# ju-liu/krylov

Hardware: AMD Instinct MI355X
Metric: CG iters/sec + SpMV GB/s (fp64, n=10M, nnz=150M); GMRES(30) iters/sec (higher is better)
Workload: dtype f64; 1 GPU; krylov.cg, 3-D 15-point stencil 216^3, one RHS per GPU, tol=0 fixed iterations; n=10077696, nnz=149770936, index=int32, rhs_per_gpu=1, parallelism=rhs-shard x1, launch=one GPU

## Files before the change

include/krylov_hip.h:

```cpp
#ifndef KRYLOV_HIP_H
#define KRYLOV_HIP_H

#include <stdint.h>

#ifdef __cplusplus
extern "C" {
#endif

typedef struct kry_ctx kry_ctx;
typedef struct kry_csr kry_csr;
typedef struct kry_vec kry_vec;
typedef struct kry_cg kry_cg;
typedef struct kry_gmres kry_gmres;
typedef struct kry_minres kry_minres;
typedef struct kry_comm kry_comm;
typedef struct kry_prog kry_prog;
typedef struct kry_tri kry_tri;
typedef struct kry_precond kry_precond;

enum { KRY_F32 = 1, KRY_F64 = 2 };
enum { KRY_I32 = 1, KRY_I64 = 2 };

enum {
  KRY_OK = 0,
  KRY_EINVAL = -1,
  KRY_ENOMEM = -2,
  KRY_EDEVICE = -3,
  KRY_EINVARIANT = -4,
  KRY_EUNSUPPORTED = -5,
  KRY_ESINGULAR = -6,
  KRY_ENONFINITE = -7,
  KRY_ECOMM = -8
};

int kry_version(void);
const char *kry_last_error(void);
const char *kry_build_id(void);
int kry_device_count(int *count);
int kry_ctx_create(int device, kry_ctx **out);
int kry_ctx_destroy(kry_ctx *ctx);
int kry_ctx_synchronize(kry_ctx *ctx);

int kry_mem_stats(int64_t *out);
int kry_mem_release(void);

int kry_csr_create(kry_ctx *ctx, int64_t n, int64_t nnz, const void *indptr,
                   const void *indices, const void *data, int dtype, int itype,
                   kry_csr **out);
int kry_csr_destroy(kry_csr *A);
int kry_csr_create_like(kry_ctx *ctx, const kry_csr *like, int64_t n, int64_t nnz, const void *indptr,
                        const void *indices, const void *data, int dtype, int itype, kry_csr **out);
int kry_csr_create_ex(kry_ctx *ctx, int64_t n, int64_t nnz, const void *indptr, const void *indices,
                      const void *data, int dtype, int itype, int renumber, kry_csr **out);
int kry_csr_permute(kry_ctx *ctx, const kry_csr *A, const kry_vec *src, kry_vec *dst, int to_operator);
int kry_csr_compare(const kry_csr *A, const kry_csr *B, int64_t *out);
int kry_spmv_op(kry_ctx *ctx, kry_csr *A, kry_vec *x, kry_vec *y);
int kry_rcm_plan(int64_t n, int64_t nnz, const void *indptr, const void *indices, int itype, int64_t wlimit,
                 int64_t *info, int32_t *perm);
int kry_rcm_device(kry_ctx *ctx, int64_t n, int64_t nnz, const int32_t *indptr, const int32_t *indices, int64_t wlimit,
                   int64_t *info, int32_t *perm);
int kry_rs_plan(int64_t n, int64_t nnz, const void *indptr, const void *indices, int itype, int64_t *info,
                int32_t *widths, uint32_t *colrank);
int kry_csr_layout(int64_t n, const void *indptr, int itype, int64_t *nslices,
                   int64_t *nslots, int64_t *nirregular);
int kry_dia_plan(int64_t n, int64_t nnz, const void *indptr, const void *indices, int itype, int64_t *info,
                 int32_t *widths, int32_t *offsets, uint64_t *masks);
int kry_dia_uniform_plan(int64_t n, int64_t nnz, const void *indptr, const void *indices, const void *data, int dtype,
                         int itype, int64_t *info, int32_t *flags, void *values);
int kry_pair_plan(int64_t n, int64_t nnz, const void *indptr, const void *indices, int itype, int64_t *info,
                  int32_t *widths, int32_t *cbase, uint16_t *deltas);
int kry_cb_plan(int64_t n, int64_t nnz, const void *indptr, const void *indices, int itype, int64_t *info,
                int64_t *gptr);
#define KRY_CSR_INFO_LEN 16
int kry_csr_info_n(const kry_csr *A, int64_t *info, int32_t len);
int kry_csr_info(const kry_csr *A, int64_t *info);

int kry_vec_create(kry_ctx *ctx, int64_t n, int32_t k, int dtype, kry_vec **out);
int kry_vec_destroy(kry_vec *v);
int kry_vec_upload(kry_vec *v, const void *host);
int kry_vec_download(kry_vec *v, void *host);

int kry_spmv(kry_ctx *ctx, kry_csr *A, kry_vec *x, kry_vec *y);
int kry_dot(kry_ctx *ctx, kry_vec *x, kry_vec *y, kry_vec *w, double *out);
int kry_axpy(kry_ctx *ctx, const double *alpha, kry_vec *x, kry_vec *y);
int kry_vec_lincomb(kry_ctx *ctx, int form, kry_vec *z, kry_vec *x, kry_vec *y, kry_vec *w,
                    const double *a, const double *b);
int kry_prog_create(kry_ctx *ctx, int32_t nregs, int32_t k, int32_t cap, kry_prog **out);
int kry_prog_destroy(kry_prog *p);
int kry_prog_set(kry_prog *p, int32_t r, const double *vals);
int kry_prog_get(kry_prog *p, int32_t r, double *vals);
int kry_prog_begin(kry_prog *p);
int kry_prog_end(kry_prog *p, int32_t steps, int32_t *done, int32_t *midstep, double *rows);
int kry_prog_scalar(kry_prog *p, int32_t op, int32_t d, int32_t a, int32_t b, int32_t c, int32_t e, double value,
                    int32_t step);
int kry_prog_dot(kry_prog *p, kry_vec *x, kry_vec *y, kry_vec *w, int32_t d, int32_t step);
int kry_prog_lincomb(kry_prog *p, int32_t form, kry_vec *z, kry_vec *x, kry_vec *y, kry_vec *w, int32_t ra, double sa,
                     int32_t rb, double sb, int32_t step);
int kry_prog_spmv(kry_prog *p, kry_csr *A, kry_vec *x, kry_vec *y, int32_t step);
int kry_prog_check(kry_prog *p, int32_t r, int32_t mode, int32_t step);
int kry_prog_rowscale(kry_prog *p, int32_t mul, kry_vec *z, kry_vec *x, kry_vec *d, int32_t step);
int kry_prog_permute(kry_prog *p, const kry_csr *A, const kry_vec *src, kry_vec *dst, int32_t to_operator,
                     int32_t step);
int kry_prog_trisolve(kry_prog *p, const kry_tri *T, const kry_vec *y, kry_vec *x, int32_t step);

int kry_tri_plan(int64_t n, int64_t nnz, const void *indptr, const void *indices, int itype, int lower, int64_t *info,
                 int32_t *level, int32_t *order, int32_t *launch, int32_t *widths);
int kry_tri_create(kry_ctx *ctx, int64_t n, int64_t nnz, const void *indptr, const void *indices, const void *data,
                   int dtype, int itype, int lower, kry_tri **out);
int kry_tri_plan_ordered(int64_t n, int64_t nnz, const void *indptr, const void *indices, int itype, int lower,
                         const int32_t *rank, int64_t *info, int32_t *level, int32_t *order, int32_t *launch,
                         int32_t *widths);
int kry_tri_create_ordered(kry_ctx *ctx, int64_t n, int64_t nnz, const void *indptr, const void *indices,
                           const void *data, int dtype, int itype, int lower, const int32_t *rank, kry_tri **out);
int kry_color_plan(int64_t n, int64_t nnz, const void *indptr, const void *indices, int itype, int64_t *info,
                   int32_t *color, int32_t *perm);
int kry_tri_destroy(kry_tri *T);
int kry_tri_info(const kry_tri *T, int64_t *info);
int kry_tri_solve(kry_ctx *ctx, const kry_tri *T, const kry_vec *y, kry_vec *x);

int kry_ilu0_plan(int64_t n, int64_t nnz, const void *indptr, const void *indices, int itype, int64_t *info,
                  int32_t *level, int32_t *order, int32_t *launch, int64_t *diag);
int kry_isai_lower(kry_ctx *ctx, int64_t n, int64_t nnz, const void *indptr, const void *indices, const void *data,
                   int dtype, int itype, void *values, int64_t *info);
int kry_precond_add_isai(kry_precond *P, const kry_csr *W, const kry_csr *T, int32_t sweeps, const kry_vec *scale);
int kry_ilu0_factor(kry_ctx *ctx, int64_t n, int64_t nnz, const void *indptr, const void *indices, const void *data,
                    int dtype, int itype, void *values, int64_t *info);
int kry_precond_create(kry_ctx *ctx, int64_t n, int dtype, kry_precond **out);
int kry_precond_destroy(kry_precond *P);
int kry_precond_add_tri(kry_precond *P, const kry_tri *T);
int kry_precond_add_scale(kry_precond *P, const kry_vec *d);
int kry_precond_fuse(kry_precond *P);
int kry_precond_info(const kry_precond *P, int64_t *info);
int kry_precond_apply(kry_ctx *ctx, const kry_precond *P, const kry_vec *x, kry_vec *y);
int kry_prog_precond(kry_prog *p, const kry_precond *P, const kry_vec *x, kry_vec *y, int32_t step);
int kry_cg_set_precond(kry_cg *s, int32_t slot, const kry_precond *P);
int kry_gmres_set_precond(kry_gmres *s, int32_t slot, const kry_precond *P);
int kry_minres_set_precond(kry_minres *s, int32_t slot, const kry_precond *P);

int kry_lartg(kry_ctx *ctx, int64_t count, int dtype, const void *f, const void *g,
              void *c, void *s, void *r);

int kry_cg_create(kry_ctx *ctx, kry_csr *A, int32_t k, int dtype, kry_cg **out);
int kry_cg_destroy(kry_cg *s);
int kry_cg_set_preconditioners(kry_cg *s, kry_csr *M, kry_csr *Ml);
int kry_cg_start(kry_cg *s, kry_vec *b, kry_vec *x0, kry_vec *w, double *rho0);
int kry_cg_set_criterion(kry_cg *s, const double *criterion);
int kry_cg_run(kry_cg *s, int32_t max_steps, int32_t *steps_done, double *resnorms);
int kry_cg_preferred_chunk(kry_cg *s, int32_t *steps);
int kry_cg_path(kry_cg *s, int32_t *info);
int kry_cg_update_path(kry_cg *s, int32_t *info);
int kry_cg_defer_info(kry_cg *s, int32_t *D, int64_t *bytes);
int kry_cg_residual(kry_cg *s, double *resnorm);
int kry_cg_get(kry_cg *s, int which, void *host);
int kry_cg_scalars(kry_cg *s, double *out);

int kry_gmres_create(kry_ctx *ctx, kry_csr *A, int32_t k, int dtype, int32_t maxiter,
// ... 50 lines not shown
```

krylov_amd/_lib.py:

```python
import atexit
import ctypes
import os
import threading
import weakref

import numpy as np

from .errors import exception_for

_HERE = os.path.dirname(os.path.abspath(__file__))
LIB_PATH = os.path.join(_HERE, "libkrylov_hip.so")
if os.environ.get("KRYLOV_LIB"):
    LIB_PATH = os.environ["KRYLOV_LIB"]

KRY_F32, KRY_F64 = 1, 2
KRY_I32, KRY_I64 = 1, 2

KRY_OK = 0
KRY_EINVAL = -1
KRY_ENOMEM = -2
KRY_EDEVICE = -3
KRY_EINVARIANT = -4
KRY_EUNSUPPORTED = -5
KRY_ESINGULAR = -6
KRY_ENONFINITE = -7
KRY_ECOMM = -8

PROF_SPMV, PROF_UPDATE, PROF_MGS, PROF_OTHER = 0, 1, 2, 3

if not os.path.exists(LIB_PATH):
    raise ImportError(
        f"{LIB_PATH} is missing: build it with `python -c 'import __graft_entry__ as g; g.build()'` "
        "or `make -C krylov_amd/csrc` (hipcc, gfx950). krylov_amd has no CPU fallback."
    )

lib = ctypes.CDLL(LIB_PATH)
HOST_ONLY = not hasattr(lib, "kry_ctx_create")

_vp = ctypes.c_void_p
_pvp = ctypes.POINTER(ctypes.c_void_p)
_i32 = ctypes.c_int32
_i64 = ctypes.c_int64
_int = ctypes.c_int
_dp = ctypes.POINTER(ctypes.c_double)
_ip32 = ctypes.POINTER(ctypes.c_int32)
_ip64 = ctypes.POINTER(ctypes.c_int64)

_SIGNATURES = {
    "kry_device_count": [ctypes.POINTER(_int)],
    "kry_ctx_create": [_int, _pvp],
    "kry_ctx_destroy": [_vp],
    "kry_ctx_synchronize": [_vp],
    "kry_csr_create": [_vp, _i64, _i64, _vp, _vp, _vp, _int, _int, _pvp],
    "kry_csr_destroy": [_vp],
    "kry_csr_create_ex": [_vp, _i64, _i64, _vp, _vp, _vp, _int, _int, _int, _pvp],
    "kry_csr_create_like": [_vp, _vp, _i64, _i64, _vp, _vp, _vp, _int, _int, _pvp],
    "kry_csr_permute": [_vp, _vp, _vp, _vp, _int],
    "kry_csr_compare": [_vp, _vp, _ip64],
    "kry_spmv_op": [_vp, _vp, _vp, _vp],
    "kry_rcm_plan": [ctypes.c_int64, ctypes.c_int64, _vp, _vp, _int, ctypes.c_int64, _ip64, _vp],
    "kry_rs_plan": [ctypes.c_int64, ctypes.c_int64, _vp, _vp, _int, _ip64, _vp, _vp],
    "kry_rcm_device": [_vp, ctypes.c_int64, ctypes.c_int64, _vp, _vp, ctypes.c_int64, _ip64, _vp],
    "kry_csr_layout": [_i64, _vp, _int, _ip64, _ip64, _ip64],
    "kry_dia_plan": [ctypes.c_int64, ctypes.c_int64, _vp, _vp, _int, _ip64, _vp, _vp, _vp],
    "kry_dia_uniform_plan": [ctypes.c_int64, ctypes.c_int64, _vp, _vp, _vp, _int, _int, _ip64, _vp, _vp],
    "kry_pair_plan": [ctypes.c_int64, ctypes.c_int64, _vp, _vp, _int, _ip64, _vp, _vp, _vp],
    "kry_cb_plan": [ctypes.c_int64, ctypes.c_int64, _vp, _vp, _int, _ip64, _vp],
    "kry_csr_info": [_vp, _ip64],
    "kry_csr_info_n": [_vp, _ip64, _i32],
    "kry_vec_create": [_vp, _i64, _i32, _int, _pvp],
    "kry_vec_destroy": [_vp],
    "kry_vec_upload": [_vp, _vp],
    "kry_vec_download": [_vp, _vp],
    "kry_spmv": [_vp, _vp, _vp, _vp],
    "kry_dot": [_vp, _vp, _vp, _vp, _dp],
    "kry_axpy": [_vp, _dp, _vp, _vp],
    "kry_lartg": [_vp, _i64, _int, _vp, _vp, _vp, _vp, _vp],
    "kry_cg_create": [_vp, _vp, _i32, _int, _pvp],
    "kry_cg_destroy": [_vp],
    "kry_cg_start": [_vp, _vp, _vp, _vp, _dp],
    "kry_cg_set_criterion": [_vp, _dp],
    "kry_cg_run": [_vp, _i32, _ip32, _dp],
    "kry_cg_preferred_chunk": [_vp, _ip32],
    "kry_cg_path": [_vp, _ip32],
    "kry_cg_update_path": [_vp, _ip32],
    "kry_cg_defer_info": [_vp, _ip32, _ip64],
    "kry_minres_update_path": [_vp, _ip32],
    "kry_cg_residual": [_vp, _dp],
    "kry_cg_get": [_vp, _int, _vp],
    "kry_cg_scalars": [_vp, _dp],
    "kry_vec_lincomb": [_vp, _int, _vp, _vp, _vp, _vp, _dp, _dp],
    "kry_cg_set_preconditioners": [_vp, _vp, _vp],
    "kry_gmres_set_preconditioners": [_vp, _vp, _vp, _vp],
    "kry_minres_set_preconditioners": [_vp, _vp, _vp, _vp],
    "kry_gmres_create": [_vp, _vp, _i32, _int, _i32, _i32, _pvp],
    "kry_gmres_destroy": [_vp],
    "kry_gmres_start": [_vp, _vp, _vp, _vp, _dp],
    "kry_gmres_set_criterion": [_vp, _dp],
    "kry_gmres_run": [_vp, _i32, _ip32, _dp, _ip32],
    "kry_trsv_upper": [_vp, _i32, _i32, ctypes.c_int, _dp, _dp, _dp],
    "kry_householder": [_vp, _vp, _vp, _dp],
    "kry_gmres_solution": [_vp],
    "kry_gmres_residual": [_vp, _dp],
    "kry_gmres_get": [_vp, _int, _vp],
    "kry_gmres_xk_device": [_vp, _vp],
    "kry_gmres_path": [_vp, _ip32],
    "kry_minres_create": [_vp, _vp, _i32, _int, _pvp],
    "kry_minres_destroy": [_vp],
    "kry_minres_start": [_vp, _vp, _vp, _vp, _dp],
    "kry_minres_set_criterion": [_vp, _dp],
    "kry_minres_run": [_vp, _i32, _ip32, _dp, _ip32],
    "kry_minres_residual": [_vp, _dp],
    "kry_minres_get": [_vp, _int, _vp],
    "kry_comm_unique_id": [_vp],
    "kry_comm_create": [_vp, _i32, _i32, _vp, _pvp],
    "kry_comm_destroy": [_vp],
    "kry_comm_abort": [_vp],
    "kry_comm_create_all": [_vp, _i32, _vp],
    "kry_comm_allreduce": [_vp, _dp, _i32],
    "kry_comm_info": [_vp, _vp, _vp],
    "kry_cg_attach_comm": [_vp, _vp, _i32, _i32],
    "kry_gmres_attach_comm": [_vp, _vp, _i32, _i32],
    "kry_minres_attach_comm": [_vp, _vp, _i32, _i32],
    "kry_timer_start": [_vp],
    "kry_timer_stop": [_vp, _dp],
    "kry_profile_enable": [_vp, _int],
    "kry_profile_select": [_vp, ctypes.c_uint32, ctypes.c_int32],
    "kry_profile_read": [_vp, _int, _ip64, _dp],
    "kry_prog_create": [_vp, _i32, _i32, _i32, _pvp],
    "kry_prog_destroy": [_vp],
    "kry_prog_set": [_vp, _i32, _dp],
    "kry_prog_get": [_vp, _i32, _dp],
    "kry_prog_begin": [_vp],
    "kry_prog_end": [_vp, _i32, _ip32, _ip32, _dp],
    "kry_prog_scalar": [_vp, _i32, _i32, _i32, _i32, _i32, _i32, ctypes.c_double, _i32],
    "kry_prog_dot": [_vp, _vp, _vp, _vp, _i32, _i32],
    "kry_prog_lincomb": [_vp, _i32, _vp, _vp, _vp, _vp, _i32, ctypes.c_double, _i32, ctypes.c_double, _i32],
    "kry_prog_spmv": [_vp, _vp, _vp, _vp, _i32],
    "kry_prog_check": [_vp, _i32, _i32, _i32],
    "kry_prog_rowscale": [_vp, _i32, _vp, _vp, _vp, _i32],
    "kry_prog_permute": [_vp, _vp, _vp, _vp, _i32, _i32],
    "kry_prog_trisolve": [_vp, _vp, _vp, _vp, _i32],
    "kry_tri_plan": [ctypes.c_int64, ctypes.c_int64, _vp, _vp, _int, _int, _ip64, _vp, _vp, _vp, _vp],
    "kry_tri_create": [_vp, _i64, _i64, _vp, _vp, _vp, _int, _int, _int, _pvp],
    "kry_tri_plan_ordered": [ctypes.c_int64, ctypes.c_int64, _vp, _vp, _int, _int, _vp, _ip64, _vp, _vp, _vp, _vp],
    "kry_tri_create_ordered": [_vp, _i64, _i64, _vp, _vp, _vp, _int, _int, _int, _vp, _pvp],
    "kry_color_plan": [ctypes.c_int64, ctypes.c_int64, _vp, _vp, _int, _ip64, _vp, _vp],
    "kry_tri_destroy": [_vp],
# ... 52 lines not shown

def dtype_code(dt):
    dt = np.dtype(dt)
    if dt == np.float64:
        return KRY_F64
    if dt == np.float32:
        return KRY_F32
    raise TypeError(f"the MI355X path computes in float32/float64, not {dt}")


def itype_code(dt):
    dt = np.dtype(dt)
    if dt == np.int32:
        return KRY_I32
    if dt == np.int64:
        return KRY_I64
    raise TypeError(f"CSR index arrays must be int32 or int64, not {dt}")


def ptr(a):
    assert a.flags.c_contiguous
    return ctypes.c_void_p(a.ctypes.data)


def dptr(a):
    assert a.dtype == np.float64 and a.flags.c_contiguous
    return a.ctypes.data_as(_dp)


def device_count():
    c = _int(0)
    check(lib.kry_device_count(ctypes.byref(c)))
    return c.value


def memory_stats():
    out = np.zeros(6, dtype=np.int64)
    check(lib.kry_mem_stats(out.ctypes.data_as(_ip64)))
    keys = ("bytes_in_use", "bytes_cached", "reuses", "device_mallocs", "retire_syncs", "enabled")
    return {k: int(v) for k, v in zip(keys, out)}


def empty_cache():
    check(lib.kry_mem_release())


def dia_plan(indptr, indices):
    indptr = np.ascontiguousarray(indptr)
    indices = np.ascontiguousarray(indices, dtype=indptr.dtype)
    n, nnz = indptr.shape[0] - 1, indices.shape[0]
    info = np.zeros(4, dtype=np.int64)
    ip64 = info.ctypes.data_as(ctypes.POINTER(ctypes.c_int64))
    check(lib.kry_dia_plan(n, nnz, ptr(indptr), ptr(indices), itype_code(indptr.dtype), ip64, None, None, None))
    if not info[0]:
        return None
    cols = int(info[2]) // 128
    widths = np.zeros(int(info[1]), dtype=np.int32)
    offsets = np.zeros(cols, dtype=np.int32)
    masks = np.zeros(2 * cols, dtype=np.uint64)
    check(lib.kry_dia_plan(n, nnz, ptr(indptr), ptr(indices), itype_code(indptr.dtype), ip64, ptr(widths),
                           ptr(offsets), ptr(masks)))
    return {"slices": int(info[1]), "slots": int(info[2]), "max_width": int(info[3]), "widths": widths,
            "offsets": offsets, "masks": masks}


def dia_uniform_plan(indptr, indices, data):
    indptr = np.ascontiguousarray(indptr)
    indices = np.ascontiguousarray(indices, dtype=indptr.dtype)
    data = np.ascontiguousarray(data)
    n, nnz = indptr.shape[0] - 1, indices.shape[0]
    assert data.shape[0] == nnz
    info = np.zeros(3, dtype=np.int64)
    ip64 = info.ctypes.data_as(ctypes.POINTER(ctypes.c_int64))
    args = (n, nnz, ptr(indptr), ptr(indices), ptr(data), dtype_code(data.dtype), itype_code(indptr.dtype), ip64)
    check(lib.kry_dia_uniform_plan(*args, None, None))
    if not info[0]:
        return None
    flags = np.zeros(int(info[1]), dtype=np.int32)
    values = np.zeros(int(info[1]), dtype=data.dtype)
    check(lib.kry_dia_uniform_plan(*args, ptr(flags), ptr(values)))
    return {"cols": int(info[1]), "uniform": int(info[2]), "flags": flags, "values": values}


def pair_plan(indptr, indices):
    indptr = np.ascontiguousarray(indptr)
    indices = np.ascontiguousarray(indices, dtype=indptr.dtype)
    n, nnz = indptr.shape[0] - 1, indices.shape[0]
    info = np.zeros(4, dtype=np.int64)
    ip64 = info.ctypes.data_as(ctypes.POINTER(ctypes.c_int64))
    check(lib.kry_pair_plan(n, nnz, ptr(indptr), ptr(indices), itype_code(indptr.dtype), ip64, None, None, None))
    if not info[0]:
        return None
    slots = int(info[2])
    widths = np.zeros(int(info[1]), dtype=np.int32)
    cbase = np.zeros(slots // 128, dtype=np.int32)
    deltas = np.zeros(slots, dtype=np.uint16)
    check(lib.kry_pair_plan(n, nnz, ptr(indptr), ptr(indices), itype_code(indptr.dtype), ip64, ptr(widths),
                            ptr(cbase), ptr(deltas)))
    return {"slices": int(info[1]), "slots": slots, "max_width": int(info[3]), "widths": widths, "cbase": cbase,
            "deltas": deltas}


def cb_plan(indptr, indices):
    indptr = np.ascontiguousarray(indptr)
    indices = np.ascontiguousarray(indices, dtype=indptr.dtype)
    n, nnz = indptr.shape[0] - 1, indices.shape[0]
    info = np.zeros(4, dtype=np.int64)
    ip64 = info.ctypes.data_as(ctypes.POINTER(ctypes.c_int64))
    check(lib.kry_cb_plan(n, nnz, ptr(indptr), ptr(indices), itype_code(indptr.dtype), ip64, None))
    if not info[0]:
        return None
    nb, ng = int(info[1]), int(info[3])
    gptr = np.zeros(nb * ng + 1, dtype=np.int64)
    check(lib.kry_cb_plan(n, nnz, ptr(indptr), ptr(indices), itype_code(indptr.dtype), ip64, ptr(gptr)))
    return {"nb": nb, "cols": int(info[2]), "ng": ng, "gptr": gptr}


def rcm_plan(indptr, indices, wlimit=0):
    indptr = np.ascontiguousarray(indptr)
    indices = np.ascontiguousarray(indices, dtype=indptr.dtype)
    n, nnz = indptr.shape[0] - 1, indices.shape[0]
    info = np.zeros(2, dtype=np.int64)
    perm = np.zeros(max(n, 1), dtype=np.int32)
    check(lib.kry_rcm_plan(n, nnz, ptr(indptr), ptr(indices), itype_code(indptr.dtype), int(wlimit),
                           info.ctypes.data_as(ctypes.POINTER(ctypes.c_int64)), ptr(perm)))
    if not info[0]:
        return None
    return perm[:n], int(info[1])


def rs_plan(indptr, indices):
    indptr = np.ascontiguousarray(indptr)
    indices = np.ascontiguousarray(indices, dtype=indptr.dtype)
    n, nnz = indptr.shape[0] - 1, indices.shape[0]
    info = np.zeros(4, dtype=np.int64)
    ip64 = info.ctypes.data_as(ctypes.POINTER(ctypes.c_int64))
    check(lib.kry_rs_plan(n, nnz, ptr(indptr), ptr(indices), itype_code(indptr.dtype), ip64, None, None))
    if not info[0]:
        return None
    widths = np.zeros(int(info[1]), dtype=np.int32)
    colrank = np.zeros(int(info[2]), dtype=np.uint32)
    check(lib.kry_rs_plan(n, nnz, ptr(indptr), ptr(indices), itype_code(indptr.dtype), ip64, ptr(widths),
                          ptr(colrank)))
    return {"slices": int(info[1]), "slots": int(info[2]), "max_width": int(info[3]), "widths": widths,
            "colrank": colrank}


def tri_plan(indptr, indices, lower=True, rank=None):
    indptr = np.ascontiguousarray(indptr)
    indices = np.ascontiguousarray(indices, dtype=indptr.dtype)
    n, nnz = indptr.shape[0] - 1, indices.shape[0]
    info = np.zeros(5, dtype=np.int64)
    ip64 = info.ctypes.data_as(ctypes.POINTER(ctypes.c_int64))
    head = (n, nnz, ptr(indptr), ptr(indices), itype_code(indptr.dtype), 1 if lower else 0)
    if rank is None:
        plan, args = lib.kry_tri_plan, head + (ip64,)
    else:
        rank = np.ascontiguousarray(rank, dtype=np.int32)
        if rank.shape != (n,):
            raise ValueError("rank must have one entry per row")
        plan, args = lib.kry_tri_plan_ordered, head + (ptr(rank), ip64)
    check(plan(*args, None, None, None, None))
    level = np.zeros(n, dtype=np.int32)
    order = np.zeros(n, dtype=np.int32)
    launch = np.zeros(int(info[1]) + 1, dtype=np.int32)
    widths = np.zeros(int(info[2]), dtype=np.int32)
# ... 94 lines not shown
```

krylov_amd/csrc/abi_core.hip:

```cpp
#include <algorithm>
#include <atomic>
#include <climits>
#include <condition_variable>
#include <cstring>
#include <map>
#include <mutex>
#include <thread>
#include <chrono>
#include <unordered_map>

#include "device.hpp"
#include "host_image.hpp"

using namespace kry;

namespace kry {

constexpr size_t kAllocSlack = 256;

namespace {

struct BlockKey {
  int device;
  size_t bytes;
// ... 280 lines not shown
  }
  void *tmp = dev_alloc(bytes + 16);
  try {
    permute_rows(A, src, tmp, k, esize, false, st);
    host_xfer(host, tmp, bytes, hipMemcpyDeviceToHost, st);
  } catch (...) {
    dev_free(tmp);
    throw;
  }
  dev_free(tmp);
}

ProfScope::ProfScope(kry_ctx *c, int kernel_id) : ctx(c), id(kernel_id) {
  if (!((ctx->profile >> kernel_id) & 1u)) return;
  if (ctx->prof_calls[kernel_id]++ % ctx->prof_every != 0) return;
  if (ctx->ev_used == ctx->ev_pool.size()) {
    hipEvent_t a, b;
    KRY_HIP(hipEventCreate(&a));
    KRY_HIP(hipEventCreate(&b));
    ctx->ev_pool.emplace_back(a, b);
    ctx->ev_ids.push_back(0);
  }
  auto &pr = ctx->ev_pool[ctx->ev_used];
  ctx->ev_ids[ctx->ev_used] = id;
  KRY_HIP(hipEventRecord(pr.first, ctx->stream));
  e1 = pr.second;
}

ProfScope::~ProfScope() {
  if (!e1) return;
  (void)hipEventRecord(e1, ctx->stream);
  ctx->ev_used++;
}



template <typename V>
struct OpDot {
  const V *x, *y;
  const double *w;
  int k;
  __device__ __forceinline__ void operator()(int64_t e, int64_t N, double (&acc)[Vec16<V>::W]) const {
    constexpr int W = Vec16<V>::W;
    V a[W], b[W];
    VIO<V>::load(x, e, N, a);
    VIO<V>::load(y, e, N, b);
#pragma unroll
    for (int v = 0; v < W; ++v)
      if (e + v < N)
        acc[v] += w ? dterm_w((double)a[v], w[(e + v) / k], (double)b[v]) : dterm((double)a[v], (double)b[v]);
  }
};

template <typename V>
struct OpAxpy {
  const V *x;
  V *y;
  const double *alpha;
  int k;
  __device__ __forceinline__ void operator()(int64_t e, int64_t N, double (&)[Vec16<V>::W]) const {
    constexpr int W = Vec16<V>::W;
    V a[W], b[W];
    VIO<V>::load(x, e, N, a);
    VIO<V>::load(y, e, N, b);
#pragma unroll
    for (int v = 0; v < W; ++v) {
      const V t = (V)alpha[(e + v) & (k - 1)] * a[v];
      b[v] = b[v] + t;
    }
    VIO<V>::store(y, e, N, b);
  }
};

template <typename T>
__global__ void lartg_kernel(int64_t count, const T *f, const T *g, T *c, T *s, T *r) {
  const int64_t i = (int64_t)blockIdx.x * blockDim.x + threadIdx.x;
  if (i < count) lartg<T>(f[i], g[i], c[i], s[i], r[i]);
}

}

extern "C" {

int kry_version(void) { return 111; }

#ifndef KRY_BUILD_ID
#define KRY_BUILD_ID "unknown"
#endif
const char *kry_build_id(void) { return KRY_BUILD_ID; }

int kry_device_count(int *count) {
  KRY_API_BEGIN
  KRY_REQUIRE(count, KRY_EINVAL, "null count");
  int c = 0;
  hipError_t e = hipGetDeviceCount(&c);
  *count = (e == hipSuccess) ? c : 0;
  KRY_API_END
}

int kry_mem_stats(int64_t *out) {
  KRY_API_BEGIN
  KRY_REQUIRE(out, KRY_EINVAL, "null out");
  kry::mem_stats(out);
  KRY_API_END
}

int kry_mem_release(void) {
  KRY_API_BEGIN
  kry::mem_release();
  KRY_API_END
}

int kry_ctx_create(int device, kry_ctx **out) {
  KRY_API_BEGIN
  KRY_REQUIRE(out, KRY_EINVAL, "null out");
  int c = 0;
  hipError_t e = hipGetDeviceCount(&c);
  KRY_REQUIRE(e == hipSuccess && c > 0, KRY_EDEVICE, "no HIP device available");
  KRY_REQUIRE(device >= 0 && device < c, KRY_EINVAL, "device index out of range");
  KRY_HIP(hipSetDevice(device));
  hipDeviceProp_t prop;
  KRY_HIP(hipGetDeviceProperties(&prop, device));
  KRY_REQUIRE(std::strncmp(prop.gcnArchName, "gfx950", 6) == 0, KRY_EDEVICE,
              std::string("libkrylov_hip is built for gfx950 only; found ") + prop.gcnArchName);
  auto *ctx = new kry_ctx();
  ctx->device = device;
  KRY_HIP(hipStreamCreateWithFlags(&ctx->stream, hipStreamNonBlocking));
  KRY_HIP(hipEventCreate(&ctx->t0));
  KRY_HIP(hipEventCreate(&ctx->t1));
  *out = ctx;
  KRY_API_END
}

int kry_ctx_destroy(kry_ctx *ctx) {
  KRY_API_BEGIN
  if (!ctx) return KRY_OK;
  (void)hipSetDevice(ctx->device);
  (void)hipStreamSynchronize(ctx->stream);
  for (auto &p : ctx->ev_pool) {
    (void)hipEventDestroy(p.first);
    (void)hipEventDestroy(p.second);
  }
  (void)hipEventDestroy(ctx->t0);
  (void)hipEventDestroy(ctx->t1);
  dev_free(ctx->scratch);
  if (ctx->pinned) (void)hipHostFree(ctx->pinned);
  (void)hipStreamDestroy(ctx->stream);
  delete ctx;
  KRY_API_END
}

int kry_ctx_synchronize(kry_ctx *ctx) {
  KRY_API_BEGIN
  KRY_REQUIRE(ctx, KRY_EINVAL, "null ctx");
  KRY_HIP(hipStreamSynchronize(ctx->stream));
  KRY_API_END
}

int kry_csr_info_n(const kry_csr *A, int64_t *info, int32_t len) {
  KRY_API_BEGIN
  KRY_REQUIRE(A && (info || len == 0) && len >= 0, KRY_EINVAL, "bad argument");
  const int64_t all[KRY_CSR_INFO_LEN] = {A->nslices,   A->nslots,    A->nirregular,        A->compact ? 1 : 0,
                                         A->cb_nb,      A->dia ? 1 : 0, A->dia_nslots,     A->sp ? 1 : 0,
                                         A->sp_nslots,  A->rs ? 1 : 0, A->rs_nslots,     A->renumbered ? 1 : 0,
                                         A->rcm_levels, A->dia ? A->dia_nuniform : 0,
                                         A->dia ? (A->dia_nslots / kDiaSlice - A->dia_nuniform) * kDiaSlice *
                                                      (int64_t)dsize(A->dtype)
                                                : 0,
                                         A->dia && dia_lean_on(A) ? 1 : 0};
  for (int i = 0; i < len && i < KRY_CSR_INFO_LEN; ++i) info[i] = all[i];
  KRY_API_END
}

int kry_csr_info(const kry_csr *A, int64_t *info) { return kry_csr_info_n(A, info, 5); }

}

namespace {
struct UploadTrace {
  bool on;
  std::chrono::steady_clock::time_point t;
  UploadTrace() {
    const char *e = getenv("KRY_UPLOAD_TRACE");
    on = e && atoi(e) != 0;
    t = std::chrono::steady_clock::now();
  }
  void mark(const char *what) {
    if (!on) return;
    const auto now = std::chrono::steady_clock::now();
    fprintf(stderr, "kry_csr_create %-28s %8.1f ms\n", what, std::chrono::duration<double, std::milli>(now - t).count());
    t = now;
  }
};

uint64_t perm_fingerprint(const std::vector<int32_t> &p) {
  uint64_t h = 1469598103934665603ull;
  for (int32_t v : p) {
    h ^= (uint32_t)v;
    h *= 1099511628211ull;
  }
  return h;
}


template <typename I, typename MV>
void csr_upload(kry_csr *A, const I *ip, const I *ix, const MV *dv, const std::vector<int32_t> *like_perm,
                bool renumber) {
  hipStream_t st = A->ctx->stream;
  const int64_t n = A->n, nnz = A->nnz;
  const bool may_renumber = renumber && !env_off("KRY_RENUMBER");
  UploadTrace tr;
  int dres = 0;
  if constexpr (sizeof(I) == 4) {
    if (!like_perm && n > 0 && nnz > 0 && !env_off("KRY_DEVICE_BUILD")) {
      DeviceCsrFlags df;
      dres = device_image_build(A, ip, ix, dv, may_renumber, &df);
      tr.mark("device build (H2D + SELL-64 + DIA)");
      if (dres == 1) return;
    }
  }
  if (dres == 0) check_csr(n, nnz, ip, ix);
  std::vector<int32_t> own;
  const std::vector<int32_t> *perm = like_perm;
  if (perm) {
    KRY_REQUIRE((int64_t)perm->size() == n, KRY_EINVAL, "renumbering of another size");
  } else if (sizeof(I) == 4 && may_renumber && scattered(n, ip, ix)) {
    const char *we = getenv("KRY_RCM_WLIMIT");
    const int64_t wlimit = we ? std::max<int64_t>(1, atoll(we)) : std::max<int64_t>(int64_t(1) << 16, n / 32);
    int r = -1;
    if constexpr (sizeof(I) == 4) {
      if (!env_off("KRY_RCM_DEVICE")) {
        void *dip = dev_alloc((size_t)(n + 1) * 4);
        void *dix = dev_alloc((size_t)std::max<int64_t>(nnz, 1) * 4);
        try {
          host_xfer(dip, ip, (size_t)(n + 1) * 4, hipMemcpyHostToDevice, st);
          if (nnz) host_xfer(dix, ix, (size_t)nnz * 4, hipMemcpyHostToDevice, st);
          r = rcm_order_device(A->ctx, n, static_cast<const int32_t *>(dip), static_cast<const int32_t *>(dix), wlimit,
                               own, &A->rcm_levels);
        } catch (...) {
          dev_free(dip);
          dev_free(dix);
          throw;
        }
        dev_free(dip);
        dev_free(dix);
      }
    }
    if (r < 0) r = rcm_order(n, ip, ix, wlimit, own, &A->rcm_levels) ? 1 : 0;
    if (r == 1) perm = &own;
    tr.mark("RCM order");
  }
  hvec<I> ip2, ix2;
  hvec<MV> dv2;
  if (perm) {
    renumber_csr(n, ip, ix, dv, *perm, ip2, ix2, dv2);
    ip = ip2.data();
    ix = ix2.data();
    dv = dv2.data();
    A->renumbered = true;
    A->perm_host = *perm;
    A->perm_hash = perm_fingerprint(A->perm_host);
    std::vector<int32_t> inv(n);
    for (int64_t r = 0; r < n; ++r) inv[A->perm_host[r]] = (int32_t)r;
    A->perm = dev_alloc((size_t)n * 4 + 4);
    A->iperm = dev_alloc((size_t)n * 4 + 4);
    KRY_HIP(hipMemcpyAsync(A->perm, A->perm_host.data(), (size_t)n * 4, hipMemcpyHostToDevice, st));
    KRY_HIP(hipMemcpyAsync(A->iperm, inv.data(), (size_t)n * 4, hipMemcpyHostToDevice, st));
    KRY_HIP(hipStreamSynchronize(st));
    tr.mark("renumbered CSR + perm H2D");
  }
  if (dres < 2) {
    std::vector<int64_t> sptr;
    std::vector<int32_t> width;
    sell_plan(n, ip, &sptr, &width, &A->nslices, &A->nslots, &A->nirregular);
    A->max_width = 0;
    for (int32_t w : width) A->max_width = std::max(A->max_width, w);
    hvec<I> sidx;
    hvec<MV> sval;
    sell_fill(n, ip, ix, dv, sptr, width, sidx, sval);
    tr.mark("SELL-64 plan + fill");
    A->sptr = dev_alloc(sptr.size() * 8);
    A->swidth = dev_alloc(width.size() * 4 + 4);
    const char *cenv = getenv("KRY_SELL_COMPACT");
    hvec<uint16_t> sdelta;
    std::vector<int32_t> scbase;
    A->compact = sizeof(I) == 4 && !(cenv && atoi(cenv) == 0) && A->nslots > 0 &&
                 compact_fill(sptr, width, sidx, sdelta, scbase);
    if (A->compact) {
      A->sdelta = dev_alloc(sdelta.size() * 2);
      A->scbase = dev_alloc(scbase.size() * 4);
      KRY_HIP(hipMemcpyAsync(A->sdelta, sdelta.data(), sdelta.size() * 2, hipMemcpyHostToDevice, st));
      KRY_HIP(hipMemcpyAsync(A->scbase, scbase.data(), scbase.size() * 4, hipMemcpyHostToDevice, st));
    } else {
      A->sidx = dev_alloc(sidx.size() * sizeof(I));
      KRY_HIP(hipMemcpyAsync(A->sidx, sidx.data(), sidx.size() * sizeof(I), hipMemcpyHostToDevice, st));
    }
    A->sval = dev_alloc(sval.size() * sizeof(MV));
    KRY_HIP(hipMemcpyAsync(A->sptr, sptr.data(), sptr.size() * 8, hipMemcpyHostToDevice, st));
    if (!width.empty()) KRY_HIP(hipMemcpyAsync(A->swidth, width.data(), width.size() * 4, hipMemcpyHostToDevice, st));
    KRY_HIP(hipMemcpyAsync(A->sval, sval.data(), sval.size() * sizeof(MV), hipMemcpyHostToDevice, st));
    KRY_HIP(hipStreamSynchronize(st));
    release_later(sidx);
    release_later(sval);
    release_later(sdelta);
    tr.mark("compact image + H2D");
  }
  const char *denv = getenv("KRY_SPMV_DIA");
  if (dres != 2 && !(denv && atoi(denv) == 0)) {
    DiaHost<MV> dh;
    if (dia_build(n, ip, ix, dv, A->nslots, dh, !env_off("KRY_DIA_UNIFORM"))) {
      A->dia = true;
      A->dia_nuniform = dh.nuniform;
      A->dia_nslices = (int64_t)dh.width.size();
      A->dia_nslots = dh.sptr.back();
      A->dia_max_width = dh.max_width;
      A->dia_sptr = dev_alloc(dh.sptr.size() * 8);
      A->dia_width = dev_alloc(dh.width.size() * 4 + 4);
      A->dia_off = dev_alloc(dh.off.size() * 4);
      A->dia_mask = dev_alloc(dh.mask.size() * 8);
      A->dia_val = dev_alloc(dh.val.size() * sizeof(MV));
      A->dia_uflag = dev_alloc(dh.uflag.size() * 4);
      A->dia_uval = dev_alloc(dh.uval.size() * sizeof(MV));
      KRY_HIP(hipMemcpyAsync(A->dia_sptr, dh.sptr.data(), dh.sptr.size() * 8, hipMemcpyHostToDevice, st));
      KRY_HIP(hipMemcpyAsync(A->dia_width, dh.width.data(), dh.width.size() * 4, hipMemcpyHostToDevice, st));
      KRY_HIP(hipMemcpyAsync(A->dia_off, dh.off.data(), dh.off.size() * 4, hipMemcpyHostToDevice, st));
      KRY_HIP(hipMemcpyAsync(A->dia_mask, dh.mask.data(), dh.mask.size() * 8, hipMemcpyHostToDevice, st));
      KRY_HIP(hipMemcpyAsync(A->dia_val, dh.val.data(), dh.val.size() * sizeof(MV), hipMemcpyHostToDevice, st));
      KRY_HIP(hipMemcpyAsync(A->dia_uflag, dh.uflag.data(), dh.uflag.size() * 4, hipMemcpyHostToDevice, st));
      KRY_HIP(hipMemcpyAsync(A->dia_uval, dh.uval.data(), dh.uval.size() * sizeof(MV), hipMemcpyHostToDevice, st));
      KRY_HIP(hipStreamSynchronize(st));
      release_later(dh.val);
    }
    tr.mark("DIA image + H2D");
  }
  const char *cbenv = getenv("KRY_SPMV_CB");
  if (!A->dia && !A->renumbered && !(cbenv && atoi(cbenv) == 0)) {
    CbHost<MV> cb;
    if (cb_build(n, ip, ix, dv, cb)) {
      A->cb_nb = cb.nb;
      A->cb_cols = cb.cols;
      A->cb_ng = cb.ng;
      A->cb_gptr = dev_alloc(cb.gptr.size() * 8);
      A->cb_roff = dev_alloc(cb.roff.size() * 2);
      A->cb_col = dev_alloc(cb.col.size() * 4);
      A->cb_val = dev_alloc(cb.val.size() * sizeof(MV));
      KRY_HIP(hipMemcpyAsync(A->cb_gptr, cb.gptr.data(), cb.gptr.size() * 8, hipMemcpyHostToDevice, st));
      KRY_HIP(hipMemcpyAsync(A->cb_roff, cb.roff.data(), cb.roff.size() * 2, hipMemcpyHostToDevice, st));
      KRY_HIP(hipMemcpyAsync(A->cb_col, cb.col.data(), cb.col.size() * 4, hipMemcpyHostToDevice, st));
      KRY_HIP(hipMemcpyAsync(A->cb_val, cb.val.data(), cb.val.size() * sizeof(MV), hipMemcpyHostToDevice, st));
      KRY_HIP(hipStreamSynchronize(st));
      release_later(cb.val);
      release_later(cb.col);
      release_later(cb.roff);
    }
    tr.mark("column-blocked image + H2D");
  }
  const char *penv = getenv("KRY_SPMV_PAIR");
  if (!A->dia && A->cb_nb == 0 && !A->renumbered && !(penv && atoi(penv) == 0)) {
    PairHost<MV> ph;
    if (pair_build(n, ip, ix, dv, A->nslots, ph)) {
      A->sp = true;
      A->sp_nslices = (int64_t)ph.width.size();
      A->sp_nslots = ph.sptr.back();
      A->sp_max_width = ph.max_width;
      A->sp_sptr = dev_alloc(ph.sptr.size() * 8);
      A->sp_width = dev_alloc(ph.width.size() * 4 + 4);
      A->sp_cbase = dev_alloc(ph.cbase.size() * 4);
      A->sp_delta = dev_alloc(ph.delta.size() * 2);
      A->sp_val = dev_alloc(ph.val.size() * sizeof(MV));
      KRY_HIP(hipMemcpyAsync(A->sp_sptr, ph.sptr.data(), ph.sptr.size() * 8, hipMemcpyHostToDevice, st));
      KRY_HIP(hipMemcpyAsync(A->sp_width, ph.width.data(), ph.width.size() * 4, hipMemcpyHostToDevice, st));
      KRY_HIP(hipMemcpyAsync(A->sp_cbase, ph.cbase.data(), ph.cbase.size() * 4, hipMemcpyHostToDevice, st));
      KRY_HIP(hipMemcpyAsync(A->sp_delta, ph.delta.data(), ph.delta.size() * 2, hipMemcpyHostToDevice, st));
      KRY_HIP(hipMemcpyAsync(A->sp_val, ph.val.data(), ph.val.size() * sizeof(MV), hipMemcpyHostToDevice, st));
      KRY_HIP(hipStreamSynchronize(st));
      release_later(ph.val);
      release_later(ph.delta);
    }
    tr.mark("paired image + H2D");
  }
  if (!A->dia && A->cb_nb == 0 && !A->sp && !env_off("KRY_SPMV_RS")) {
    RsHost<MV> rh;
    if (rs_build(n, ip, ix, dv, A->nslots, rh)) {
      A->rs = true;
      A->rs_nslices = (int64_t)rh.width.size();
      A->rs_nslots = rh.sptr.back();
      A->rs_max_width = rh.max_width;
      A->rs_sptr = dev_alloc(rh.sptr.size() * 8);
      A->rs_width = dev_alloc(rh.width.size() * 4 + 4);
      A->rs_colrank = dev_alloc(rh.colrank.size() * 4);
      A->rs_val = dev_alloc(rh.val.size() * sizeof(MV));
      KRY_HIP(hipMemcpyAsync(A->rs_sptr, rh.sptr.data(), rh.sptr.size() * 8, hipMemcpyHostToDevice, st));
      KRY_HIP(hipMemcpyAsync(A->rs_width, rh.width.data(), rh.width.size() * 4, hipMemcpyHostToDevice, st));
      KRY_HIP(hipMemcpyAsync(A->rs_colrank, rh.colrank.data(), rh.colrank.size() * 4, hipMemcpyHostToDevice, st));
      KRY_HIP(hipMemcpyAsync(A->rs_val, rh.val.data(), rh.val.size() * sizeof(MV), hipMemcpyHostToDevice, st));
      KRY_HIP(hipStreamSynchronize(st));
      release_later(rh.colrank);
      release_later(rh.val);
    }
    tr.mark("rank-sorted image + H2D");
  }
  if (A->nirregular > 0 && !A->indptr) {
    A->indptr = dev_alloc((n + 1) * sizeof(I));
    A->indices = dev_alloc((nnz + 1) * sizeof(I));
    A->data = dev_alloc((nnz + 1) * sizeof(MV));
    host_xfer(A->indptr, ip, (n + 1) * sizeof(I), hipMemcpyHostToDevice, st);
    if (nnz) {
      host_xfer(A->indices, ix, nnz * sizeof(I), hipMemcpyHostToDevice, st);
      host_xfer(A->data, dv, nnz * sizeof(MV), hipMemcpyHostToDevice, st);
    }
  }
  KRY_HIP(hipStreamSynchronize(st));
  release_later(ix2);
  release_later(dv2);
  tr.mark("CSR copy + final sync");
}
}

static void csr_free(kry_csr *A) {
  void *bufs[] = {A->sptr,   A->swidth,   A->sidx,     A->sval,     A->indptr,    A->indices,
                  A->data,   A->sdelta,   A->scbase,   A->cb_gptr,  A->cb_roff,   A->cb_col,
                  A->cb_val, A->dia_sptr, A->dia_width, A->dia_off, A->dia_mask, A->dia_val,
                  A->sp_sptr, A->sp_width, A->sp_cbase, A->sp_delta, A->sp_val,
                  A->rs_sptr, A->rs_width, A->rs_colrank, A->rs_val, A->perm, A->iperm,
                  A->dia_uflag, A->dia_uval};
  for (void *b : bufs) dev_free(b);
}

extern "C" {

static kry_csr *csr_create(kry_ctx *ctx, int64_t n, int64_t nnz, const void *indptr, const void *indices,
                           const void *data, int dtype, int itype, const kry_csr *like, bool renumber = true) {
  KRY_REQUIRE(ctx && indptr && (nnz == 0 || (indices && data)), KRY_EINVAL, "null argument");
  KRY_REQUIRE(n >= 0 && nnz >= 0, KRY_EINVAL, "negative size");
  KRY_REQUIRE(dtype == KRY_F32 || dtype == KRY_F64, KRY_EINVAL, "dtype must be f32 or f64");
  KRY_REQUIRE(itype == KRY_I32 || itype == KRY_I64, KRY_EINVAL, "itype must be i32 or i64");
  if (itype == KRY_I32) KRY_REQUIRE(nnz < (int64_t(1) << 31) && n < (int64_t(1) << 31), KRY_EINVAL,
                                    "int32 indices cannot address this matrix");
  KRY_REQUIRE(!like || like->n == n, KRY_EINVAL, "the operator to renumber like has another size");
  KRY_HIP(hipSetDevice(ctx->device));
  auto *A = new kry_csr();
  A->ctx = ctx;
  A->n = n;
  A->nnz = nnz;
  A->dtype = dtype;
  A->itype = itype;
  static const int32_t zi32 = 0;
  static const int64_t zi64 = 0;
  static const double zd = 0;
  const std::vector<int32_t> *lp = like && like->renumbered ? &like->perm_host : nullptr;
  try {
    const void *ix = nnz ? indices : (itype == KRY_I32 ? (const void *)&zi32 : (const void *)&zi64);
    const void *dv = nnz ? data : (const void *)&zd;
    if (itype == KRY_I32 && dtype == KRY_F64)
      csr_upload(A, static_cast<const int32_t *>(indptr), static_cast<const int32_t *>(ix), static_cast<const double *>(dv), lp, renumber);
    else if (itype == KRY_I32)
      csr_upload(A, static_cast<const int32_t *>(indptr), static_cast<const int32_t *>(ix), static_cast<const float *>(dv), lp, renumber);
    else if (dtype == KRY_F64)
      csr_upload(A, static_cast<const int64_t *>(indptr), static_cast<const int64_t *>(ix), static_cast<const double *>(dv), lp, renumber);
    else
      csr_upload(A, static_cast<const int64_t *>(indptr), static_cast<const int64_t *>(ix), static_cast<const float *>(dv), lp, renumber);
  } catch (...) {
    csr_free(A);
    delete A;
    throw;
  }
  return A;
}

int kry_csr_create(kry_ctx *ctx, int64_t n, int64_t nnz, const void *indptr, const void *indices,
                   const void *data, int dtype, int itype, kry_csr **out) {
  KRY_API_BEGIN
  KRY_REQUIRE(out, KRY_EINVAL, "null argument");
  *out = csr_create(ctx, n, nnz, indptr, indices, data, dtype, itype, nullptr);
  KRY_API_END
}

int kry_csr_create_ex(kry_ctx *ctx, int64_t n, int64_t nnz, const void *indptr, const void *indices,
                      const void *data, int dtype, int itype, int renumber, kry_csr **out) {
  KRY_API_BEGIN
  KRY_REQUIRE(out, KRY_EINVAL, "null argument");
  *out = csr_create(ctx, n, nnz, indptr, indices, data, dtype, itype, nullptr, renumber != 0);
  KRY_API_END
}

int kry_csr_create_like(kry_ctx *ctx, const kry_csr *like, int64_t n, int64_t nnz, const void *indptr,
                        const void *indices, const void *data, int dtype, int itype, kry_csr **out) {
  KRY_API_BEGIN
  KRY_REQUIRE(out && like, KRY_EINVAL, "null argument");
  *out = csr_create(ctx, n, nnz, indptr, indices, data, dtype, itype, like);
  KRY_API_END
}

int kry_csr_compare(const kry_csr *A, const kry_csr *B, int64_t *out) {
  KRY_API_BEGIN
  KRY_REQUIRE(A && B && out, KRY_EINVAL, "null argument");
  KRY_HIP(hipSetDevice(A->ctx->device));
  KRY_HIP(hipDeviceSynchronize());
  int64_t nd = 0, mask = 0;
  int item = 0;
  auto note = [&](bool differ) {
    if (differ) {
      ++nd;
      mask |= int64_t(1) << item;
    }
    ++item;
  };
  const int64_t scal[][2] = {{A->nslices, B->nslices}, {A->nslots, B->nslots}, {A->nirregular, B->nirregular},
                             {A->max_width, B->max_width}, {A->compact, B->compact}, {A->dia, B->dia},
                             {A->dia_nslices, B->dia_nslices}, {A->dia_nslots, B->dia_nslots},
                             {A->dia_max_width, B->dia_max_width}};
  for (auto &p : scal) note(p[0] != p[1]);
  auto buf = [&](const void *a, const void *b, size_t bytes) {
    if (!a || !b) {
      note(a != b);
      return;
    }
    std::vector<char> ha(bytes), hb(bytes);
    if (bytes) {
      KRY_HIP(hipMemcpy(ha.data(), a, bytes, hipMemcpyDeviceToHost));
      KRY_HIP(hipMemcpy(hb.data(), b, bytes, hipMemcpyDeviceToHost));
    }
    note(bytes && std::memcmp(ha.data(), hb.data(), bytes) != 0);
  };
  if (nd == 0) {
    const size_t ds = dsize(A->dtype), is = isize(A->itype);
    buf(A->sptr, B->sptr, (A->nslices + 1) * 8);
    buf(A->swidth, B->swidth, A->nslices * 4);
    buf(A->sval, B->sval, (A->nslots + 256) * ds);
    buf(A->sidx, B->sidx, A->compact ? 0 : (A->nslots + 256) * is);
    buf(A->sdelta, B->sdelta, A->compact ? (A->nslots + 256) * 2 : 0);
    buf(A->scbase, B->scbase, A->compact ? (A->nslots / kSlice + 16) * 4 : 0);
    const int64_t dc = A->dia_nslots / kDiaSlice + kDiaPad;
    buf(A->dia_sptr, B->dia_sptr, A->dia ? (A->dia_nslices + 1) * 8 : 0);
    buf(A->dia_width, B->dia_width, A->dia ? A->dia_nslices * 4 : 0);
    buf(A->dia_off, B->dia_off, A->dia ? dc * 4 : 0);
    buf(A->dia_mask, B->dia_mask, A->dia ? dc * 16 : 0);
    buf(A->dia_val, B->dia_val, A->dia ? (A->dia_nslots + 256) * ds : 0);
    buf(A->indptr, B->indptr, A->nirregular ? (A->n + 1) * is : 0);
    buf(A->indices, B->indices, A->nirregular ? A->nnz * is : 0);
    buf(A->data, B->data, A->nirregular ? A->nnz * ds : 0);
    note(A->dia_nuniform != B->dia_nuniform);
    buf(A->dia_uflag, B->dia_uflag, A->dia ? dc * 4 : 0);
    buf(A->dia_uval, B->dia_uval, A->dia ? dc * ds : 0);
  }
  out[0] = nd;
  out[1] = mask;
  KRY_API_END
}

int kry_csr_permute(kry_ctx *ctx, const kry_csr *A, const kry_vec *src, kry_vec *dst, int to_operator) {
  KRY_API_BEGIN
  KRY_REQUIRE(ctx && A && src && dst, KRY_EINVAL, "null argument");
  KRY_REQUIRE(src->n == A->n && dst->n == A->n && src->k == dst->k && src->dtype == dst->dtype, KRY_EINVAL,
              "shape mismatch");
  KRY_REQUIRE(src != dst, KRY_EINVAL, "src and dst must differ");
  KRY_HIP(hipSetDevice(ctx->device));
  permute_rows(A, src->d, dst->d, src->k, dsize(src->dtype), to_operator != 0, ctx->stream);
  KRY_API_END
}

int kry_csr_destroy(kry_csr *A) {
  KRY_API_BEGIN
  if (!A) return KRY_OK;
  (void)hipSetDevice(A->ctx->device);
  (void)hipStreamSynchronize(A->ctx->stream);
  csr_free(A);
  delete A;
  KRY_API_END
}

int kry_vec_create(kry_ctx *ctx, int64_t n, int32_t k, int dtype, kry_vec **out) {
  KRY_API_BEGIN
  KRY_REQUIRE(ctx && out, KRY_EINVAL, "null argument");
  KRY_REQUIRE(n >= 0 && k >= 1, KRY_EINVAL, "bad vector shape");
  KRY_REQUIRE(dtype == KRY_F32 || dtype == KRY_F64, KRY_EINVAL, "dtype must be f32 or f64");
  KRY_HIP(hipSetDevice(ctx->device));
  auto *v = new kry_vec();
  v->ctx = ctx;
  v->n = n;
  v->k = k;
  v->dtype = dtype;
  const size_t elems = padded_elems(n, k);
  try {
    v->d = dev_alloc(elems * dsize(dtype));
    KRY_HIP(hipMemsetAsync(v->d, 0, elems * dsize(dtype), ctx->stream));
  } catch (...) {
    delete v;
    throw;
  }
  *out = v;
  KRY_API_END
}

int kry_vec_destroy(kry_vec *v) {
  KRY_API_BEGIN
  if (!v) return KRY_OK;
  (void)hipSetDevice(v->ctx->device);
  (void)hipStreamSynchronize(v->ctx->stream);
  dev_free(v->d);
  delete v;
  KRY_API_END
}

int kry_vec_upload(kry_vec *v, const void *host) {
  KRY_API_BEGIN
  KRY_REQUIRE(v && host, KRY_EINVAL, "null argument");
  host_xfer(v->d, host, v->bytes(), hipMemcpyHostToDevice, v->ctx->stream);
  KRY_API_END
}

int kry_vec_download(kry_vec *v, void *host) {
  KRY_API_BEGIN
  KRY_REQUIRE(v && host, KRY_EINVAL, "null argument");
  host_xfer(host, v->d, v->bytes(), hipMemcpyDeviceToHost, v->ctx->stream);
  KRY_API_END
}

int kry_spmv(kry_ctx *ctx, kry_csr *A, kry_vec *x, kry_vec *y) {
  KRY_API_BEGIN
  KRY_REQUIRE(ctx && A && x && y, KRY_EINVAL, "null argument");
  KRY_REQUIRE(x->n == A->n && y->n == A->n && x->k == y->k, KRY_EINVAL, "shape mismatch");
  KRY_REQUIRE(x->dtype == y->dtype, KRY_EINVAL, "dtype mismatch");
  KRY_REQUIRE(is_pow2(x->k) && x->k <= kMaxCols, KRY_EUNSUPPORTED, "k must be a power of two <= 256");
  KRY_HIP(hipSetDevice(ctx->device));
  const int k = x->k;
  const size_t vb = (size_t)A->n * k * dsize(x->dtype) + 16;
// ... 189 lines not shown
```

krylov_amd/csrc/device.hpp:

```cpp
#pragma once

#include <type_traits>

#include "common.hpp"
#include "objects.hpp"

namespace kry {

__device__ __forceinline__ double dterm(double x, double y) { return x * y; }
__device__ __forceinline__ double dterm_w(double x, double w, double y) { return x * (w * y); }

template <typename V, int C>
__device__ __forceinline__ void vload_row(const V *p, V (&o)[C]) {
  if constexpr (sizeof(V) == 8) {
    typedef double d2 __attribute__((ext_vector_type(2)));
#pragma unroll
    for (int q = 0; q < C / 2; ++q) {
      const d2 t = reinterpret_cast<const d2 *>(p)[q];
      o[2 * q] = t.x;
      o[2 * q + 1] = t.y;
    }
  } else {
    typedef float fC __attribute__((ext_vector_type(C)));
    const fC t = *reinterpret_cast<const fC *>(p);
// ... 415 lines not shown
  for (int c = 0; c < KT; ++c) dacc[c] = 0.0;
  for (int64_t s = s_begin; s < s_end; ++s) {
    const int w = swidth[s];
    const int64_t row = s * 64 + lane;
    V acc[KT];
#pragma unroll
    for (int c = 0; c < KT; ++c) acc[c] = V(0);
    if (w >= 0) {
      const int64_t base = sptr[s];
      const I *ci = sidx + base + lane;
      const uint16_t *cd = sdelta + base + lane;
      const int *cb = scbase + (base >> 6);
      const MV *cv = sval + base + lane;
      for (int j0 = 0; j0 < w; j0 += UNR) {
        I col[UNR];
        V a[UNR];
#pragma unroll
        for (int u = 0; u < UNR; ++u) {
          const bool in = j0 + u < w;
          if constexpr (D16) {
            const unsigned d = in ? (unsigned)__builtin_nontemporal_load(cd + (int64_t)(j0 + u) * 64) : 0xFFFFu;
            const int b = in ? cb[j0 + u] : 0;
            col[u] = d != 0xFFFFu ? I(b + (int)d) : I(-1);
          } else {
            col[u] = in ? __builtin_nontemporal_load(ci + (int64_t)(j0 + u) * 64) : I(-1);
          }
          a[u] = in ? (V)__builtin_nontemporal_load(cv + (int64_t)(j0 + u) * 64) : V(0);
        }
        V xv[UNR][KT];
#pragma unroll
        for (int u = 0; u < UNR; ++u)
#pragma unroll
          for (int c = 0; c < KT; ++c) xv[u][c] = col[u] >= 0 ? bs(col[u], c) : V(0);
#pragma unroll
        for (int u = 0; u < UNR; ++u)
          if (col[u] >= 0) {
#pragma unroll
            for (int c = 0; c < KT; ++c) {
              const V p = a[u] * xv[u][c];
              acc[c] = acc[c] + p;
            }
          }
      }
    } else if (row < n) {
      for (I e = indptr[row]; e < indptr[row + 1]; ++e) {
        const I j = indices[e];
        const V a = (V)data[e];
#pragma unroll
        for (int c = 0; c < KT; ++c) {
          const V p = a * bs(j, c);
          acc[c] = acc[c] + p;
        }
      }
    }
    if (row < n) {
#pragma unroll
      for (int c = 0; c < KT; ++c) dacc[c] += epi(row, c0 + c, acc[c], bs(row, c));
    }
  }
  if (part != nullptr) {
#pragma unroll
    for (int c = 0; c < KT; ++c) red[tid * KT + c] = dacc[c];
    if (nch == 1) {
      block_tree_reduce(red, kBlock * KT, k);
      if (tid < k) part[(int64_t)g * k + tid] = red[tid];
    } else {
      __syncthreads();
      double sum = 0.0;
      if (tid < k) {
        const int cg = tid / KT, cc = tid % KT;
        for (int t = 0; t < kBlock; ++t)
          if ((int)(((int64_t)g * 4 + (t >> 6)) % nch) == cg) sum += red[t * KT + cc];
      }
      __syncthreads();
      if (tid < k) part[(int64_t)g * k + tid] = sum;
    }
  }
}


template <typename V, typename MV, int UNR, class Src, class Epi, int UNI = 1, bool LEAN = false>
__global__ __launch_bounds__(kBlock) void spmv_dia_kernel(const int64_t *__restrict__ sptr,
                                                          const int *__restrict__ swidth,
                                                          const int *__restrict__ doff,
                                                          const uint64_t *__restrict__ dmask,
                                                          const int *__restrict__ duflag,
                                                          const MV *__restrict__ duval,
                                                          const MV *__restrict__ val, int64_t nslices, int64_t n,
                                                          Src src, Epi epi, double *__restrict__ part,
                                                          const Ctrl *ctrl, int step) {
  if (halted(ctrl, step)) return;
  __shared__ double red[kBlock];
  const int tid = threadIdx.x;
  const int lane = tid & 63;
  const int wid = __builtin_amdgcn_readfirstlane(tid >> 6);
  const int g = xcd_remap(blockIdx.x, gridDim.x);
  const int64_t W = (int64_t)gridDim.x * 4;
  const int64_t m = (int64_t)g * 4 + wid;
  const int64_t s_begin = nslices * m / W, s_end = nslices * (m + 1) / W;
  const auto bs = src.template bind<1>(0);
  [[maybe_unused]] __amdgpu_buffer_rsrc_t xr;
  if constexpr (LEAN) xr = bs.pair_rsrc(n);
  [[maybe_unused]] const int lbyte = lane * 2 * (int)sizeof(V);
  double dacc = 0.0;
  V pend[2] = {V(0), V(0)};
  int64_t prow = -1;
  auto flush = [&]() {
    if (prow + 1 < n) {
      V xi[2];
      bs.pair(prow, xi);
      dacc += epi.rows2(prow, pend, xi);
    } else if (prow < n) {
      dacc += epi(prow, 0, pend[0], bs(prow, 0));
    }
  };
  for (int64_t s = s_begin; s < s_end; ++s) {
    const int w = swidth[s];
    const int64_t base = sptr[s];
    const int64_t row = s * kDiaSlice + 2 * lane;
    const int64_t c0 = base / kDiaSlice;
    const int *mo = doff + c0;
    const uint64_t *mk = dmask + 2 * c0;
    const int *mu = duflag + c0;
    const MV *mv = duval + c0;
    const MV *cv = val + base + 2 * lane;
    V acc0 = V(0), acc1 = V(0);
    for (int j0 = 0; j0 < w; j0 += UNR) {
      int off[UNR], uf[UNR];
      uint64_t me[UNR], md[UNR];
      MV uv[UNR];
#pragma unroll
      for (int u = 0; u < UNR; ++u) {
        off[u] = mo[j0 + u];
        me[u] = mk[2 * (j0 + u)];
        md[u] = mk[2 * (j0 + u) + 1];
        uf[u] = UNI == 1 ? mu[j0 + u] : UNI / 2;
        uv[u] = UNI == 0 ? MV(0) : mv[j0 + u];
      }
      bool stream = false;
#pragma unroll
      for (int u = 0; u < UNR; ++u) stream = stream || (j0 + u < w && uf[u] == 0);
      MV a[UNR][2];
      if (UNI == 2 || (UNI == 1 && !stream)) {
#pragma unroll
        for (int u = 0; u < UNR; ++u) {
          a[u][0] = uv[u];
          a[u][1] = uv[u];
        }
      } else {
#pragma unroll
        for (int u = 0; u < UNR; ++u) {
          if (j0 + u < w && uf[u] == 0) {
            pload_nt<MV>(cv + (int64_t)(j0 + u) * kDiaSlice, a[u]);
          } else {
            a[u][0] = uv[u];
            a[u][1] = uv[u];
          }
        }
      }
      bool on0[UNR], on1[UNR];
      V xv[UNR][2];
#pragma unroll
      for (int u = 0; u < UNR; ++u) {
        if constexpr (LEAN) {
          on0[u] = __builtin_amdgcn_inverse_ballot_w64(j0 + u < w ? me[u] : 0);
          on1[u] = __builtin_amdgcn_inverse_ballot_w64(j0 + u < w ? md[u] : 0);
          bs.pair_at(xr, xpair_byte<V>(s * kDiaSlice + off[u]) + lbyte, xv[u]);
        } else {
          on0[u] = j0 + u < w && ((me[u] >> lane) & 1u) != 0;
          on1[u] = j0 + u < w && ((md[u] >> lane) & 1u) != 0;
          bs.pair((on0[u] || on1[u]) ? row + off[u] : 0, xv[u]);
        }
      }
      if (j0 == 0 && prow >= 0) {
        __builtin_amdgcn_sched_barrier(0);
        flush();
        __builtin_amdgcn_sched_barrier(0);
      }
#pragma unroll
      for (int u = 0; u < UNR; ++u) {
        const V p0 = (V)a[u][0] * xv[u][0];
        const V p1 = (V)a[u][1] * xv[u][1];
        const V t0 = acc0 + p0;
        const V t1 = acc1 + p1;
        acc0 = on0[u] ? t0 : acc0;
        acc1 = on1[u] ? t1 : acc1;
      }
    }
    if (w == 0 && prow >= 0) flush();
    pend[0] = acc0;
    pend[1] = acc1;
    prow = row;
  }
  if (prow >= 0) flush();
  if (part != nullptr) {
    red[tid] = dacc;
    block_tree_reduce(red, kBlock, 1);
    if (tid == 0) part[g] = red[0];
  }
}

template <typename V, typename MV, int UNR, class Src, class Epi>
__global__ __launch_bounds__(kBlock) void spmv_pair_kernel(const int64_t *__restrict__ sptr,
// ... 720 lines not shown
      int r0 = 0, r1 = 0;
      if (has) {
        r0 = roff[(int64_t)b * n + row];
        r1 = (tid == kCbRows - 1 || row + 1 >= n) ? len : (int)roff[(int64_t)b * n + row + 1];
      }
      cb_segment<VEC, V, MV>(s0, len, r0, r1, col, val, bs, prod, acc[o], tid);
    }
  }
  double dacc = 0.0;
#pragma unroll
  for (int o = 0; o < kCbMaxOwn; ++o) {
    const int64_t g = g0 + (int64_t)blockIdx.x + (int64_t)o * gridDim.x;
    if (g >= g1) break;
    const int64_t row = g * kCbRows + tid;
    if (row < n) dacc += epi(row, 0, acc[o], bs(row, 0));
  }
  if (part != nullptr) {
    __syncthreads();
    red[tid] = dacc;
    block_tree_reduce(red, kBlock, 1);
    if (tid == 0) part[blockIdx.x] = red[0];
  }
}

template <typename V, typename MV, typename I, int KT, int UNR, bool D16, class Src, class Epi>
int launch_sell_img(const kry_csr *A, int k, Src src, Epi epi, double *part, const Ctrl *ctrl, int step,
                    hipStream_t st) {
  const int nch = k / KT;
  int64_t waves = A->nslices * nch;
  int grid = (int)((waves + 3) / 4);
  if (grid > kMaxGrid) grid = kMaxGrid;
  if (grid < 1) grid = 1;
  if (nch > 1) grid = (grid + 7) / 8 * 8;
  if (grid > kMaxGrid) grid = kMaxGrid;
  hipLaunchKernelGGL((spmv_sell_kernel<V, MV, I, KT, UNR, D16, Src, Epi>), dim3(grid), dim3(kBlock), 0, st,
                     static_cast<const int64_t *>(A->sptr), static_cast<const int *>(A->swidth),
                     static_cast<const I *>(A->sidx), static_cast<const uint16_t *>(A->sdelta),
                     static_cast<const int *>(A->scbase), static_cast<const MV *>(A->sval), A->nslices, A->n, k,
                     static_cast<const I *>(A->indptr), static_cast<const I *>(A->indices),
                     static_cast<const MV *>(A->data), src, epi, part, ctrl, step);
  return grid;
}

template <typename V, typename MV, typename I, int KT, int UNR, class Src, class Epi>
int launch_sell(const kry_csr *A, int k, Src src, Epi epi, double *part, const Ctrl *ctrl, int step,
                hipStream_t st) {
  if constexpr (sizeof(I) == 4) {
    if (A->compact) return launch_sell_img<V, MV, I, KT, UNR, true>(A, k, src, epi, part, ctrl, step, st);
  }
  return launch_sell_img<V, MV, I, KT, UNR, false>(A, k, src, epi, part, ctrl, step, st);
}

inline bool cb_vec() {
  static const bool on = [] {
    const char *e = getenv("KRY_CB_VEC");
    return !(e && atoi(e) == 0);
  }();
  return on;
}

inline bool dia_blk_off() {
  static const bool off = [] {
    const char *e = getenv("KRY_SPMV_DIA_BLK");
    return e && atoi(e) == 0;
  }();
  return off;
}

inline int rs1_on() {
  const char *e = getenv("KRY_SPMV_RS1");
  return e ? atoi(e) : 2;
}

constexpr int64_t kDiaLeanMaxBytes = 0xFFFF0000LL;
inline bool dia_lean_on(const kry_csr *A) {
  if (A->dia_lean < 0) {
    const char *e = getenv("KRY_DIA_LEAN"), *m = getenv("KRY_DIA_LEAN_MAX_BYTES");
    const int64_t cap = m ? std::min<int64_t>(kDiaLeanMaxBytes, atoll(m)) : kDiaLeanMaxBytes;
    A->dia_lean = !(e && atoi(e) == 0) && (A->n + 2) * 8 <= cap ? 1 : 0;
  }
  return A->dia_lean == 1;
}

template <typename I>
inline bool spmv_column_blocked(const kry_csr *A, int k) {
  return sizeof(I) == 4 && k == 1 && !A->dia && A->cb_nb > 0;
}

template <typename V, typename MV, typename I, class Src, class Epi>
void launch_spmv(const kry_csr *A, int k, Src src, Epi epi, double *part, int *grid_out, const Ctrl *ctrl,
                 int step, hipStream_t st) {
  KRY_REQUIRE(k >= 1 && k <= kMaxCols && is_pow2(k), KRY_EUNSUPPORTED, "k must be a power of two <= 256");
  int grid;
  if (k == 1 && A->sp) {
    grid = (int)std::max<int64_t>(1, std::min<int64_t>(kMaxGridBlk, (A->sp_nslices + 3) / 4));
    hipLaunchKernelGGL((spmv_pair_kernel<V, MV, 8, Src, Epi>), dim3(grid), dim3(kBlock), 0, st,
                       static_cast<const int64_t *>(A->sp_sptr), static_cast<const int *>(A->sp_width),
                       static_cast<const int *>(A->sp_cbase), static_cast<const uint32_t *>(A->sp_delta),
                       static_cast<const MV *>(A->sp_val), A->sp_nslices, A->n, src, epi, part, ctrl, step);
    KRY_HIP(hipGetLastError());
    if (grid_out) *grid_out = grid;
    return;
  }
  if (k == 1 && A->rs && rs1_on()) {
    grid = (int)std::max<int64_t>(1, std::min<int64_t>(kMaxGridBlk, (2 * A->rs_nslices + 3) / 4));
    auto go = [&](auto kern) {
      hipLaunchKernelGGL(kern, dim3(grid), dim3(kBlock), 0, st, static_cast<const int64_t *>(A->rs_sptr),
                         static_cast<const int *>(A->rs_width), static_cast<const uint32_t *>(A->rs_colrank),
                         static_cast<const MV *>(A->rs_val), A->rs_nslices, A->n, src, epi, part, ctrl, step);
    };
    if (rs1_on() == 2)
      go(spmv_rs1_kernel<V, MV, 16, Src, Epi>);
    else
      go(spmv_rs1_kernel<V, MV, 8, Src, Epi>);
    KRY_HIP(hipGetLastError());
    if (grid_out) *grid_out = grid;
    return;
  }
  if (k == 1 && A->rs) {
    grid = (int)std::max<int64_t>(1, std::min<int64_t>(kMaxGridBlk, (A->rs_nslices + 3) / 4));
    hipLaunchKernelGGL((spmv_rs_kernel<V, MV, 8, Src, Epi>), dim3(grid), dim3(kBlock), 0, st,
                       static_cast<const int64_t *>(A->rs_sptr), static_cast<const int *>(A->rs_width),
                       static_cast<const uint32_t *>(A->rs_colrank), static_cast<const MV *>(A->rs_val),
                       A->rs_nslices, A->n, src, epi, part, ctrl, step);
    KRY_HIP(hipGetLastError());
    if (grid_out) *grid_out = grid;
    return;
  }
  if constexpr (sizeof(I) == 4) {
    if (k == 1 && A->dia) {
      static const int dia_cap_env = [] {
        const char *e = getenv("KRY_DIA_GRID");
        return e ? std::max(1, std::min(atoi(e), kMaxGridBlk)) : 0;
      }();
      const bool allu = A->dia_nuniform > 0 && A->dia_nuniform == A->dia_nslots / kDiaSlice;
      constexpr int kDiaGridUniform = 5120;
      const int dia_cap = dia_cap_env                        ? dia_cap_env
                          : A->dia_max_width <= 8            ? kMaxGrid
                          : allu                             ? kDiaGridUniform
                                                             : kMaxGridBlk;
      grid = (int)std::max<int64_t>(1, std::min<int64_t>(dia_cap, (A->dia_nslices + 3) / 4));
      auto go = [&](auto kern) {
        hipLaunchKernelGGL(kern, dim3(grid), dim3(kBlock), 0, st, static_cast<const int64_t *>(A->dia_sptr),
                           static_cast<const int *>(A->dia_width), static_cast<const int *>(A->dia_off),
                           static_cast<const uint64_t *>(A->dia_mask), static_cast<const int *>(A->dia_uflag),
                           static_cast<const MV *>(A->dia_uval), static_cast<const MV *>(A->dia_val),
                           A->dia_nslices, A->n, src, epi, part, ctrl, step);
      };
      if (dia_lean_on(A)) {
        if (allu) go(spmv_dia_kernel<V, MV, 8, Src, Epi, 2, true>);
        else if (A->dia_nuniform == 0 && A->dia_max_width <= 8) go(spmv_dia_kernel<V, MV, 8, Src, Epi, 0, true>);
        else if (A->dia_nuniform == 0) go(spmv_dia_kernel<V, MV, 16, Src, Epi, 0, true>);
        else if (A->dia_max_width <= 8) go(spmv_dia_kernel<V, MV, 8, Src, Epi, 1, true>);
        else go(spmv_dia_kernel<V, MV, 16, Src, Epi, 1, true>);
      } else if (allu) go(spmv_dia_kernel<V, MV, 8, Src, Epi, 2>);
      else if (A->dia_nuniform == 0 && A->dia_max_width <= 8) go(spmv_dia_kernel<V, MV, 8, Src, Epi, 0>);
      else if (A->dia_nuniform == 0) go(spmv_dia_kernel<V, MV, 16, Src, Epi, 0>);
      else if (A->dia_max_width <= 8) go(spmv_dia_kernel<V, MV, 8, Src, Epi, 1>);
      else go(spmv_dia_kernel<V, MV, 16, Src, Epi, 1>);
      KRY_HIP(hipGetLastError());
      if (grid_out) *grid_out = grid;
      return;
    }
    constexpr int CPLB = 16 / (int)sizeof(V);
    if (k >= CPLB && k <= 8 && A->dia && !dia_blk_off()) {
      grid = (int)std::max<int64_t>(1, std::min<int64_t>(kMaxGridBlk, (A->dia_nslices + 3) / 4));
      auto go = [&](auto kern) {
        hipLaunchKernelGGL(kern, dim3(grid), dim3(kBlock), 0, st, static_cast<const int64_t *>(A->dia_sptr),
                           static_cast<const int *>(A->dia_width), static_cast<const int *>(A->dia_off),
                           static_cast<const uint64_t *>(A->dia_mask), static_cast<const MV *>(A->dia_val),
                           A->dia_nslices, A->n, k, src, epi, part, ctrl, step);
      };
      switch (k / CPLB) {
        case 1: go(spmv_dia_blk_kernel<V, MV, CPLB, 2, Src, Epi>); break;
        case 2: go(spmv_dia_blk_kernel<V, MV, CPLB, 4, Src, Epi>); break;
        default: go(spmv_dia_blk_kernel<V, MV, CPLB, 8, Src, Epi>); break;
      }
      KRY_HIP(hipGetLastError());
      if (grid_out) *grid_out = grid;
      return;
    }
    if (k == 1 && A->cb_nb > 0) {
      const int64_t per = (int64_t)kCbPersistGrid * kCbMaxOwn;
      grid = (int)std::min<int64_t>(A->cb_ng, kCbPersistGrid);
      int nl = 0;
      for (int64_t g0 = 0; g0 < A->cb_ng; g0 += per, ++nl) {
        const int64_t g1 = std::min<int64_t>(A->cb_ng, g0 + per);
        double *pl = part ? part + (int64_t)nl * grid : nullptr;
        auto go = [&](auto kern) {
          hipLaunchKernelGGL(kern, dim3(grid), dim3(kBlock), 0, st, (int)A->cb_nb, A->n, A->cb_ng, g0, g1,
                             static_cast<const int64_t *>(A->cb_gptr), static_cast<const uint16_t *>(A->cb_roff),
                             static_cast<const int *>(A->cb_col), static_cast<const MV *>(A->cb_val), src, epi, pl,
                             ctrl, step);
        };
        if (cb_vec()) go(spmv_cbp_kernel<true, V, MV, Src, Epi>);
        else go(spmv_cbp_kernel<false, V, MV, Src, Epi>);
      }
      KRY_HIP(hipGetLastError());
      if (grid_out) *grid_out = grid * nl;
      return;
    }
  }
  if (k >= 4 && k <= 64) {
    grid = (int)std::max<int64_t>(1, std::min<int64_t>(kMaxGrid, (A->nslices + 3) / 4));
    const bool d16 = sizeof(I) == 4 && A->compact;
    auto go = [&](auto kern) {
      hipLaunchKernelGGL(kern, dim3(grid), dim3(kBlock), 0, st, static_cast<const int64_t *>(A->sptr),
                         static_cast<const int *>(A->swidth), static_cast<const I *>(A->sidx),
                         static_cast<const uint16_t *>(A->sdelta), static_cast<const int *>(A->scbase),
                         static_cast<const MV *>(A->sval), A->nslices, A->n, k, static_cast<const I *>(A->indptr),
                         static_cast<const I *>(A->indices), static_cast<const MV *>(A->data), src, epi, part, ctrl,
                         step);
    };
    if (d16) go(spmv_sell_lg_kernel<V, MV, I, 4, 8, true, Src, Epi>);
    else go(spmv_sell_lg_kernel<V, MV, I, 4, 8, false, Src, Epi>);
    KRY_HIP(hipGetLastError());
    if (grid_out) *grid_out = grid;
    return;
  }
  switch (k) {
    case 1:
      grid = A->max_width <= 8 ? launch_sell<V, MV, I, 1, 8>(A, k, src, epi, part, ctrl, step, st)
                               : launch_sell<V, MV, I, 1, 16>(A, k, src, epi, part, ctrl, step, st);
      break;
    case 2: grid = launch_sell<V, MV, I, 2, 8>(A, k, src, epi, part, ctrl, step, st); break;
    case 4: grid = launch_sell<V, MV, I, 4, 4>(A, k, src, epi, part, ctrl, step, st); break;
    default: grid = launch_sell<V, MV, I, 8, 4>(A, k, src, epi, part, ctrl, step, st); break;
  }
  KRY_HIP(hipGetLastError());
  if (grid_out) *grid_out = grid;
// ... 43 lines not shown
```

krylov_amd/csrc/device_build.hip:

```cpp
#include <hipcub/hipcub.hpp>

#include "common.hpp"
#include "host_image.hpp"
#include "objects.hpp"

namespace kry {
namespace {

constexpr int kDb = 256;
constexpr int kDiaWMax = 64;
constexpr int kDiaLdsEnt = 8192;

enum : unsigned {
  F_INDPTR = 1u,
  F_RANGE = 2u,
  F_UNSORTED = 4u,
  F_UNSORTED_NS = 8u
};

__global__ __launch_bounds__(kDb) void csr_check_kernel(int64_t n, int64_t nnz, const int32_t *__restrict__ ip,
                                                        const int32_t *__restrict__ ix, int64_t half, unsigned *flags,
                                                        unsigned long long *far) {
  unsigned f = 0;
  unsigned long long fa = 0;
  for (int64_t r = (int64_t)blockIdx.x * kDb + threadIdx.x; r < n; r += (int64_t)gridDim.x * kDb) {
    const int32_t e0 = ip[r], e1 = ip[r + 1];
    if (e1 < e0 || e0 < 0 || (int64_t)e1 > nnz) {
      f |= F_INDPTR;
      continue;
    }
    int32_t prev = INT32_MIN;
    for (int32_t e = e0; e < e1; ++e) {
      const int32_t c = ix[e];
      if (c < 0 || (int64_t)c >= n) f |= F_RANGE;
      if (e > e0 && c <= prev) f |= F_UNSORTED;
      if (e > e0 && c < prev) f |= F_UNSORTED_NS;
      prev = c;
      const int64_t d = (int64_t)c - r;
      fa += (d > half || d < -half) ? 1u : 0u;
    }
  }
  if (f) atomicOr(flags, f);
  if (fa) atomicAdd(far, fa);
}

__device__ __forceinline__ int wave_max_i(int v) {
#pragma unroll
  for (int o = 32; o >= 1; o >>= 1) v = max(v, __shfl_xor(v, o));
  return v;
}
__device__ __forceinline__ int wave_min_i(int v) {
#pragma unroll
  for (int o = 32; o >= 1; o >>= 1) v = min(v, __shfl_xor(v, o));
  return v;
}

__global__ __launch_bounds__(kDb) void sell_plan_kernel(int64_t n, int64_t ns, const int32_t *__restrict__ ip,
                                                        int *width, long long *slots, unsigned long long *nirr,
                                                        int *maxw) {
  const int lane = threadIdx.x & 63;
  const int64_t s = ((int64_t)blockIdx.x * kDb + threadIdx.x) >> 6;
  if (s >= ns) return;
  const int64_t r = s * kSlice + lane;
  const int len = r < n ? ip[r + 1] - ip[r] : 0;
  const int w = wave_max_i(len);
  if (lane == 0) {
    const int64_t r0 = s * kSlice, r1 = r0 + kSlice < n ? r0 + kSlice : n;
    const int64_t snnz = (int64_t)ip[r1] - (int64_t)ip[r0];
    const bool irregular = (int64_t)kSlice * w > 2 * snnz + 1024 || w > (1 << 30);
    width[s] = irregular ? -1 : w;
    slots[s] = irregular ? 0 : (long long)kSlice * w;
    if (irregular) atomicAdd(nirr, 1ull);
    atomicMax(maxw, irregular ? -1 : w);
  }
}

template <typename MV>
__global__ __launch_bounds__(kDb) void sell_fill_kernel(int64_t n, int64_t ns, const int32_t *__restrict__ ip,
                                                        const int32_t *__restrict__ ix, const MV *__restrict__ dv,
                                                        const long long *__restrict__ sptr, const int *__restrict__ width,
                                                        int32_t *sidx, MV *sval, uint16_t *sdelta, int32_t *scbase,
                                                        unsigned *nocompact) {
  const int lane = threadIdx.x & 63;
// ... 73 lines not shown
      const int v = t >= d ? pre[t - d] : 0;
      __syncthreads();
      pre[t] += v;
      __syncthreads();
    }
    const int rank = total + pre[t] - head;
    if (head && rank < kDiaWMax) offs[s * kDiaWMax + rank] = buf[i];
    const int add = pre[kDb - 1];
    __syncthreads();
    total += add;
  }
  if (t == 0) {
    if ((int64_t)total * kDiaSlice > 2 * (int64_t)snnz + 2048) atomicOr(fail, 1u);
    else if (total > kDiaWMax) atomicOr(fail, 2u);
    width[s] = total;
    slots[s] = (long long)kDiaSlice * total;
    atomicMax(maxw, total);
  }
}

template <typename MV>
__global__ __launch_bounds__(kDb) void dia_fill_kernel(int64_t n, const int32_t *__restrict__ ip,
                                                       const int32_t *__restrict__ ix, const MV *__restrict__ dv,
                                                       const long long *__restrict__ sptr, const int *__restrict__ width,
                                                       const int *__restrict__ offs, int32_t *doff, uint64_t *dmask,
                                                       MV *dval, int uniform, int32_t *uflag, MV *uval,
                                                       unsigned long long *nuniform) {
  using Bits = typename std::conditional<sizeof(MV) == 8, unsigned long long, unsigned>::type;
  __shared__ int o[kDiaWMax];
  __shared__ unsigned long long msk[2 * kDiaWMax];
  const int64_t s = blockIdx.x;
  const int t = threadIdx.x;
  const int w = width[s];
  const int64_t base = sptr[s];
  const int64_t c0 = base / kDiaSlice;
  if (t < w) o[t] = offs[s * kDiaWMax + t];
  if (t < 2 * kDiaWMax) msk[t] = 0ull;
  __syncthreads();
  const int64_t r0 = s * kDiaSlice;
  if (t < kDiaSlice && r0 + t < n) {
    const int64_t r = r0 + t;
    for (int32_t e = ip[r]; e < ip[r + 1]; ++e) {
      const int off = (int)((int64_t)ix[e] - r);
      int lo = 0, hi = w;
      while (lo < hi) {
        const int mid = (lo + hi) >> 1;
        if (o[mid] < off) lo = mid + 1;
        else hi = mid;
      }
      atomicOr(&msk[2 * lo + (t & 1)], 1ull << (t >> 1));
      dval[base + (int64_t)lo * kDiaSlice + t] = dv[e];
    }
  }
  __syncthreads();
  if (t < w) {
    doff[c0 + t] = o[t];
    dmask[2 * (c0 + t)] = msk[2 * t];
    dmask[2 * (c0 + t) + 1] = msk[2 * t + 1];
  }
  if (!uniform) return;
  const int lane = t & 63;
  unsigned nu = 0;
  for (int j = t >> 6; j < w; j += kDb / 64) {
    const unsigned long long me = msk[2 * j], md = msk[2 * j + 1];
    if ((me | md) == 0ull) continue;
    const int le = me ? __ffsll((long long)me) - 1 : 64, ld = md ? __ffsll((long long)md) - 1 : 64;
    const int first = le <= ld ? 2 * le : 2 * ld + 1;
    const MV *cv = dval + base + (int64_t)j * kDiaSlice;
    const MV refv = cv[first];
    const Bits ref = __builtin_bit_cast(Bits, refv);
    const bool differ = (((me >> lane) & 1ull) && __builtin_bit_cast(Bits, cv[2 * lane]) != ref) ||
                        (((md >> lane) & 1ull) && __builtin_bit_cast(Bits, cv[2 * lane + 1]) != ref);
    if (__ballot(differ) == 0ull) {
      if (lane == 0) {
        uflag[c0 + j] = 1;
        uval[c0 + j] = refv;
      }
      ++nu;
    }
  }
  if (lane == 0 && nu) atomicAdd(nuniform, (unsigned long long)nu);
}

int grid_for_n(int64_t items, int per_block) {
  return (int)std::max<int64_t>(1, std::min<int64_t>(1 << 20, (items + per_block - 1) / per_block));
}

void exclusive_scan(const long long *cnt, long long *out, int64_t m, hipStream_t st) {
  size_t tb = 0;
  KRY_HIP(hipcub::DeviceScan::ExclusiveSum(nullptr, tb, cnt, out, (int)(m + 1), st));
  void *tmp = dev_alloc(tb + 16);
  try {
    KRY_HIP(hipcub::DeviceScan::ExclusiveSum(tmp, tb, cnt, out, (int)(m + 1), st));
  } catch (...) {
    dev_free(tmp);
    throw;
  }
  dev_free(tmp);
}

struct Tmp {
  void *p = nullptr;
  explicit Tmp(size_t b) : p(dev_alloc(b)) {}
  ~Tmp() { dev_free(p); }
  Tmp(const Tmp &) = delete;
  Tmp &operator=(const Tmp &) = delete;
  template <class T>
  T *as() const {
    return static_cast<T *>(p);
  }
  void *release() {
    void *q = p;
    p = nullptr;
    return q;
  }
};

template <typename T>
T read1(const T *d, hipStream_t st) {
  T v;
  KRY_HIP(hipMemcpyAsync(&v, d, sizeof(T), hipMemcpyDeviceToHost, st));
  KRY_HIP(hipStreamSynchronize(st));
  return v;
}

}

template <typename MV>
int device_image_build(kry_csr *A, const int32_t *ip, const int32_t *ix, const MV *dv, bool renumber_candidates,
                       DeviceCsrFlags *out) {
  hipStream_t st = A->ctx->stream;
  const int64_t n = A->n, nnz = A->nnz;
  KRY_REQUIRE(ip[0] == 0 && (int64_t)ip[n] == nnz, KRY_EINVAL, "indptr must start at 0 and end at nnz");
  Tmp dip((size_t)(n + 1) * 4 + 16), dix((size_t)nnz * 4 + 16), ddv((size_t)nnz * sizeof(MV) + 16);
  host_xfer(dip.p, ip, (size_t)(n + 1) * 4, hipMemcpyHostToDevice, st);
  host_xfer(dix.p, ix, (size_t)nnz * 4, hipMemcpyHostToDevice, st);
  host_xfer(ddv.p, dv, (size_t)nnz * sizeof(MV), hipMemcpyHostToDevice, st);
  Tmp small(256);
  KRY_HIP(hipMemsetAsync(small.p, 0, 256, st));
  unsigned *flags = small.as<unsigned>();
  unsigned long long *far = reinterpret_cast<unsigned long long *>(small.as<char>() + 16);
  const int64_t cols = std::max<int64_t>(int64_t(1) << 18, (n + 15) / 16);
  hipLaunchKernelGGL(csr_check_kernel, dim3(grid_for_n(n, kDb)), dim3(kDb), 0, st, n, nnz, dip.as<int32_t>(),
                     dix.as<int32_t>(), cols / 2, flags, far);
  KRY_HIP(hipGetLastError());
  const unsigned f = read1(flags, st);
  const unsigned long long nfar = read1(far, st);
  KRY_REQUIRE(!(f & F_INDPTR), KRY_EINVAL, "indptr must be non-decreasing");
  KRY_REQUIRE(!(f & F_RANGE), KRY_EINVAL, "column index out of range [0, n)");
  out->strictly_sorted = !(f & F_UNSORTED);
  out->sorted = !(f & F_UNSORTED_NS);
  out->scattered = n * 8 >= (int64_t(8) << 20) && nnz > 0 && (int64_t)nfar * 4 >= nnz;
  if (out->scattered && renumber_candidates) return 0;
  const int64_t ns = (n + kSlice - 1) / kSlice;
  Tmp cnt((size_t)(ns + 1) * 8 + 16);
  KRY_HIP(hipMemsetAsync(cnt.p, 0, (size_t)(ns + 1) * 8, st));
  void *swidth = dev_alloc((size_t)ns * 4 + 4);
  A->swidth = swidth;
  unsigned long long *nirr = reinterpret_cast<unsigned long long *>(small.as<char>() + 32);
  int *maxw = reinterpret_cast<int *>(small.as<char>() + 48);
  fill_kernel<int><<<1, 1, 0, st>>>(maxw, 1, -1);
  hipLaunchKernelGGL(sell_plan_kernel, dim3(grid_for_n(ns * 64, kDb)), dim3(kDb), 0, st, n, ns, dip.as<int32_t>(),
                     static_cast<int *>(swidth), cnt.as<long long>(), nirr, maxw);
  A->sptr = dev_alloc((size_t)(ns + 1) * 8);
  exclusive_scan(cnt.as<long long>(), static_cast<long long *>(A->sptr), ns, st);
  A->nslices = ns;
  A->nslots = read1(static_cast<const long long *>(A->sptr) + ns, st);
  A->nirregular = (int64_t)read1(nirr, st);
  A->max_width = read1(maxw, st);
  const int64_t slots = A->nslots;
  Tmp sidx((size_t)(slots + 256) * 4);
  A->sval = dev_alloc((size_t)(slots + 256) * sizeof(MV));
  Tmp sdelta((size_t)(slots + 256) * 2 + 16);
  Tmp scbase((size_t)(slots / kSlice + 16) * 4);
  fill_kernel<int32_t><<<grid_for_n(slots + 256, kDb), kDb, 0, st>>>(sidx.as<int32_t>(), slots + 256, -1);
  fill_kernel<MV><<<grid_for_n(slots + 256, kDb), kDb, 0, st>>>(static_cast<MV *>(A->sval), slots + 256, MV(0));
  fill_kernel<uint16_t><<<grid_for_n(slots + 256, kDb), kDb, 0, st>>>(sdelta.as<uint16_t>(), slots + 256, (uint16_t)0xFFFF);
  KRY_HIP(hipMemsetAsync(scbase.p, 0, (size_t)(slots / kSlice + 16) * 4, st));
  unsigned *nocompact = small.as<unsigned>() + 16;
  if (slots > 0)
    hipLaunchKernelGGL(sell_fill_kernel<MV>, dim3(grid_for_n(ns * 64, kDb)), dim3(kDb), 0, st, n, ns, dip.as<int32_t>(),
                       dix.as<int32_t>(), ddv.as<MV>(), static_cast<const long long *>(A->sptr),
                       static_cast<const int *>(swidth), sidx.as<int32_t>(), static_cast<MV *>(A->sval),
                       sdelta.as<uint16_t>(), scbase.as<int32_t>(), nocompact);
  KRY_HIP(hipGetLastError());
  const char *cenv = getenv("KRY_SELL_COMPACT");
  A->compact = !(cenv && atoi(cenv) == 0) && slots > 0 && read1(nocompact, st) == 0;
  if (A->compact) {
    A->sdelta = sdelta.release();
    A->scbase = scbase.release();
  } else {
    A->sidx = sidx.release();
  }
  const char *denv = getenv("KRY_SPMV_DIA");
  bool dia = out->strictly_sorted && !(denv && atoi(denv) == 0) && n > 0;
  bool host_dia = false;
  if (dia) {
    const int64_t dns = (n + kDiaSlice - 1) / kDiaSlice;
    unsigned *dfail = small.as<unsigned>() + 20;
    int *dmaxw = reinterpret_cast<int *>(small.as<char>() + 96);
    Tmp dcnt((size_t)(dns + 1) * 8 + 16), offs((size_t)dns * kDiaWMax * 4 + 16);
    KRY_HIP(hipMemsetAsync(dcnt.p, 0, (size_t)(dns + 1) * 8, st));
    Tmp dwidth((size_t)dns * 4 + 4);
    hipLaunchKernelGGL(dia_offsets_kernel, dim3((unsigned)dns), dim3(kDb), 0, st, n, dns, dip.as<int32_t>(),
                       dix.as<int32_t>(), dwidth.as<int>(), offs.as<int>(), dcnt.as<long long>(), dfail, dmaxw);
    KRY_HIP(hipGetLastError());
    const unsigned df = read1(dfail, st);
    if (df & 1u) dia = false;
    if (!(df & 1u) && (df & 2u)) host_dia = true;
    if (df == 0) {
      Tmp dsptr((size_t)(dns + 1) * 8);
      exclusive_scan(dcnt.as<long long>(), dsptr.as<long long>(), dns, st);
      const int64_t dslots = read1(dsptr.as<long long>() + dns, st);
      const int dmw = read1(dmaxw, st);
      if (!(dslots * 4 > slots * 5 + (int64_t)4 * kDiaSlice * dmw)) {
        const int64_t dcols = dslots / kDiaSlice;
        Tmp doff((size_t)(dcols + kDiaPad) * 4), dmask((size_t)2 * (dcols + kDiaPad) * 8),
            dval((size_t)(dslots + 2 * kDiaSlice) * sizeof(MV)), duflag((size_t)(dcols + kDiaPad) * 4),
            duval((size_t)(dcols + kDiaPad) * sizeof(MV));
        unsigned long long *dnuni = reinterpret_cast<unsigned long long *>(small.as<char>() + 112);
        KRY_HIP(hipMemsetAsync(duflag.p, 0, (size_t)(dcols + kDiaPad) * 4, st));
        KRY_HIP(hipMemsetAsync(duval.p, 0, (size_t)(dcols + kDiaPad) * sizeof(MV), st));
        KRY_HIP(hipMemsetAsync(doff.p, 0, (size_t)(dcols + kDiaPad) * 4, st));
        KRY_HIP(hipMemsetAsync(dmask.p, 0, (size_t)2 * (dcols + kDiaPad) * 8, st));
        KRY_HIP(hipMemsetAsync(dval.p, 0, (size_t)(dslots + 2 * kDiaSlice) * sizeof(MV), st));
        hipLaunchKernelGGL(dia_fill_kernel<MV>, dim3((unsigned)dns), dim3(kDb), 0, st, n, dip.as<int32_t>(),
                           dix.as<int32_t>(), ddv.as<MV>(), dsptr.as<const long long>(), dwidth.as<const int>(),
                           offs.as<const int>(), doff.as<int32_t>(), dmask.as<uint64_t>(), dval.as<MV>(),
                           env_off("KRY_DIA_UNIFORM") ? 0 : 1, duflag.as<int32_t>(), duval.as<MV>(), dnuni);
        KRY_HIP(hipGetLastError());
        A->dia_nuniform = (int64_t)read1(dnuni, st);
        A->dia = true;
        A->dia_nslices = dns;
        A->dia_nslots = dslots;
        A->dia_max_width = dmw;
        A->dia_sptr = dsptr.release();
        A->dia_width = dwidth.release();
        A->dia_off = doff.release();
        A->dia_mask = dmask.release();
        A->dia_val = dval.release();
        A->dia_uflag = duflag.release();
        A->dia_uval = duval.release();
      }
    }
  }
  if (A->nirregular > 0) {
    A->indptr = dip.release();
    A->indices = dix.release();
    A->data = ddv.release();
  }
  KRY_HIP(hipStreamSynchronize(st));
  return A->dia ? 1 : (host_dia ? 3 : 2);
}

template int device_image_build<double>(kry_csr *, const int32_t *, const int32_t *, const double *, bool,
                                        DeviceCsrFlags *);
template int device_image_build<float>(kry_csr *, const int32_t *, const int32_t *, const float *, bool,
                                       DeviceCsrFlags *);

}
```

krylov_amd/csrc/host_common.hpp:

```cpp
#pragma once

#include <stddef.h>
#include <stdint.h>

#include <exception>
#include <string>

#include "../../include/krylov_hip.h"

namespace kry {

constexpr int kSlice = 64;
constexpr int kDiaSlice = 128;
constexpr int kDiaPad = 32;
constexpr int kPairSlice = 128;
constexpr int kCbRows = 256;
constexpr int kRsChunk = 16;
constexpr int kTriGroupRows = 1024;

void set_error(const std::string &msg);

struct Error {
  int code;
  std::string msg;
};

#define KRY_REQUIRE(cond, code, msg)                                           \
  do {                                                                         \
    if (!(cond)) throw ::kry::Error{(code), (msg)};                            \
  } while (0)

}

#define KRY_API_BEGIN try {
#define KRY_API_END                  \
  return KRY_OK;                     \
  }                                  \
  catch (const kry::Error &e) {      \
    kry::set_error(e.msg);           \
    return e.code;                   \
  }                                  \
  catch (const std::exception &e) {  \
    kry::set_error(e.what());        \
    return KRY_EDEVICE;              \
  }
```

krylov_amd/csrc/host_image.cpp:

```cpp
#include "host_image.hpp"

#include <algorithm>
#include <atomic>
#include <climits>
#include <cstdlib>
#include <cstring>
#include <functional>
#include <thread>
#include <type_traits>

namespace kry {

static thread_local std::string g_last_error;
void set_error(const std::string &msg) { g_last_error = msg; }

template <class T>
void release_later(hvec<T> &v) {
  if (v.capacity() < (size_t(64) << 20) / sizeof(T)) {
    hvec<T>().swap(v);
    return;
  }
  auto *h = new hvec<T>();
  h->swap(v);
  std::thread([h] { delete h; }).detach();
}

template <class T>
static void par_fill(hvec<T> &v, size_t n, T val) {
  v.resize(n);
  const unsigned nt = n < (size_t(1) << 20) ? 1u : std::max(1u, std::min(16u, std::thread::hardware_concurrency()));
  if (nt == 1) {
    std::fill(v.begin(), v.end(), val);
    return;
  }
  std::vector<std::thread> th;
  for (unsigned t = 0; t < nt; ++t)
    th.emplace_back([&, t] { std::fill(v.data() + n * t / nt, v.data() + n * (t + 1) / nt, val); });
  for (auto &x : th) x.join();
}

template <typename I>
void check_csr(int64_t n, int64_t nnz, const I *ip, const I *ix) {
  KRY_REQUIRE(n >= 0 && nnz >= 0 && ip, KRY_EINVAL, "bad CSR arguments");
  KRY_REQUIRE(ip[0] == 0 && (int64_t)ip[n] == nnz, KRY_EINVAL, "indptr must start at 0 and end at nnz");
  KRY_REQUIRE(nnz == 0 || ix, KRY_EINVAL, "null indices");
  const unsigned nt = n + nnz < (int64_t(1) << 20) ? 1u : std::max(1u, std::min(16u, std::thread::hardware_concurrency()));
  std::atomic<int> bad{0};
  auto work = [&](unsigned t) {
    const int64_t r0 = n * t / nt, r1 = n * (t + 1) / nt;
    for (int64_t r = r0; r < r1; ++r)
      if (ip[r + 1] < ip[r]) {
        bad = 1;
        return;
      }
    const int64_t e0 = (int64_t)ip[r0], e1 = (int64_t)ip[r1];
    for (int64_t e = e0; e < e1; ++e)
      if (ix[e] < 0 || (int64_t)ix[e] >= n) {
        bad = 2;
        return;
      }
  };
  if (nt == 1) {
    work(0);
  } else {
    std::vector<std::thread> th;
    for (unsigned t = 0; t < nt; ++t) th.emplace_back(work, t);
    for (auto &x : th) x.join();
  }
  KRY_REQUIRE(bad != 1, KRY_EINVAL, "indptr must be non-decreasing");
  KRY_REQUIRE(bad != 2, KRY_EINVAL, "column index out of range [0, n)");
}

template <typename I>
void sell_plan(int64_t n, const I *ip, std::vector<int64_t> *sptr, std::vector<int32_t> *width,
                      int64_t *nslices, int64_t *nslots, int64_t *nirr) {
  const int64_t ns = (n + kSlice - 1) / kSlice;
  if (sptr) sptr->assign(ns + 1, 0);
  if (width) width->assign(ns, 0);
  int64_t slots = 0, irr = 0;
  for (int64_t s = 0; s < ns; ++s) {
    const int64_t r0 = s * kSlice, r1 = std::min<int64_t>(n, r0 + kSlice);
    int64_t w = 0;
    for (int64_t r = r0; r < r1; ++r) w = std::max<int64_t>(w, (int64_t)ip[r + 1] - (int64_t)ip[r]);
    const int64_t snnz = (int64_t)ip[r1] - (int64_t)ip[r0];
    const bool irregular = kSlice * w > 2 * snnz + 1024 || w > (int64_t(1) << 30);
    if (irregular) ++irr;
    if (width) (*width)[s] = irregular ? -1 : (int32_t)w;
    if (!irregular) slots += kSlice * w;
    if (sptr) (*sptr)[s + 1] = slots;
  }
  *nslices = ns;
  *nslots = slots;
// ... 102 lines not shown
          same = same && (int64_t)ix[e] - r == (int64_t)ix[e - len] - (r - 1);
        }
        if (!same)
          for (int64_t e = ip[r]; e < ip[r + 1]; ++e) o.push_back((int32_t)((int64_t)ix[e] - r));
      }
      std::sort(o.begin(), o.end());
      o.erase(std::unique(o.begin(), o.end()), o.end());
      if ((int64_t)o.size() * H > 2 * ((int64_t)ip[r1] - (int64_t)ip[r0]) + 2048) {
        ok = false;
        return;
      }
      offs[s] = o;
    }
  };
  {
    std::vector<std::thread> th;
    for (unsigned t = 0; t < nt; ++t) th.emplace_back(pass1, ns * t / nt, ns * (t + 1) / nt);
    for (auto &x : th) x.join();
  }
  if (!ok) return false;
  d.sptr.assign(ns + 1, 0);
  d.width.assign(ns, 0);
  for (int64_t s = 0; s < ns; ++s) {
    d.width[s] = (int32_t)offs[s].size();
    d.max_width = std::max(d.max_width, d.width[s]);
    d.sptr[s + 1] = d.sptr[s] + (int64_t)H * d.width[s];
  }
  const int64_t slots = d.sptr[ns];
  if (slots * 4 > sell_slots * 5 + (int64_t)4 * H * d.max_width) return false;
  const int64_t cols = slots / H;
  d.off.assign(cols + kDiaPad, 0);
  par_fill(d.mask, 2 * (cols + kDiaPad), (uint64_t)0);
  par_fill(d.val, slots + 2 * H, MV(0));
  d.uflag.assign(cols + kDiaPad, 0);
  d.uval.assign(cols + kDiaPad, MV(0));
  std::atomic<int64_t> nuniform{0};
  auto pass2 = [&](int64_t sa, int64_t sb) {
    int64_t nu = 0;
    for (int64_t s = sa; s < sb; ++s) {
      const std::vector<int32_t> &o = offs[s];
      const int64_t base = d.sptr[s], c0 = base / H;
      for (size_t j = 0; j < o.size(); ++j) d.off[c0 + j] = o[j];
      const int64_t r0 = s * H, r1 = std::min<int64_t>(n, r0 + H);
      for (int64_t r = r0; r < r1; ++r) {
        const int rl = (int)(r - r0);
        size_t j = 0;
        for (int64_t e = ip[r]; e < ip[r + 1]; ++e) {
          const int32_t off = (int32_t)((int64_t)ix[e] - r);
          while (o[j] != off) ++j;
          d.mask[2 * (c0 + j) + (rl & 1)] |= uint64_t(1) << (rl >> 1);
          d.val[base + (int64_t)j * H + rl] = dv[e];
          ++j;
        }
      }
      if (!uniform) continue;
      for (size_t j = 0; j < o.size(); ++j) {
        const uint64_t m[2] = {d.mask[2 * (c0 + j)], d.mask[2 * (c0 + j) + 1]};
        const MV *v = d.val.data() + base + (int64_t)j * H;
        int first = -1;
        bool same = true;
        for (int rl = 0; rl < H && same; ++rl) {
          if (!((m[rl & 1] >> (rl >> 1)) & 1u)) continue;
          if (first < 0) first = rl;
          same = value_bits(v[rl]) == value_bits(v[first]);
        }
        if (first >= 0 && same) {
          d.uflag[c0 + j] = 1;
          d.uval[c0 + j] = v[first];
          ++nu;
        }
      }
    }
    nuniform += nu;
  };
  {
    std::vector<std::thread> th;
    for (unsigned t = 0; t < nt; ++t) th.emplace_back(pass2, ns * t / nt, ns * (t + 1) / nt);
    for (auto &x : th) x.join();
  }
  d.nuniform = nuniform.load();
  return true;
}


namespace {
struct Team {
  unsigned nt;
  std::vector<std::thread> th;
  std::atomic<unsigned> gen{0}, left{0};
  std::atomic<bool> quit{false};
  std::function<void(unsigned)> job;
  explicit Team(unsigned want) : nt(std::max(1u, want)) {
    for (unsigned t = 1; t < nt; ++t)
      th.emplace_back([this, t] {
        unsigned seen = 0;
        for (;;) {
          unsigned g;
          while ((g = gen.load(std::memory_order_acquire)) == seen) {
            if (quit.load(std::memory_order_acquire)) return;
            std::this_thread::yield();
          }
          seen = g;
          job(t);
          left.fetch_sub(1, std::memory_order_acq_rel);
        }
      });
  }
  void run(const std::function<void(unsigned)> &f) {
    if (nt == 1) {
      f(0);
      return;
    }
    job = f;
    left.store(nt - 1, std::memory_order_release);
    gen.fetch_add(1, std::memory_order_acq_rel);
    f(0);
    while (left.load(std::memory_order_acquire) != 0) std::this_thread::yield();
  }
  ~Team() {
    quit.store(true, std::memory_order_release);
    for (auto &x : th) x.join();
  }
};

template <typename I>
void bfs_expand(Team &tm, const I *ip, const I *ix, const int32_t *front, int64_t nf, int32_t next,
                std::atomic<int32_t> *level, std::vector<std::vector<int32_t>> &loc, std::vector<int32_t> &out) {
  tm.run([&](unsigned t) {
    auto &v = loc[t];
    v.clear();
    const int64_t a = nf * t / tm.nt, b = nf * (t + 1) / tm.nt;
    for (int64_t q = a; q < b; ++q) {
      const int32_t u = front[q];
      for (int64_t e = ip[u]; e < ip[u + 1]; ++e) {
        const int32_t w = (int32_t)ix[e];
        int32_t expect = -1;
        if (level[w].load(std::memory_order_relaxed) == -1 &&
            level[w].compare_exchange_strong(expect, next, std::memory_order_relaxed))
          v.push_back(w);
      }
    }
  });
  out.clear();
  for (auto &v : loc) out.insert(out.end(), v.begin(), v.end());
}
}

template <typename I>
bool scattered(int64_t n, const I *ip, const I *ix) {
  if (n * 8 < (int64_t(8) << 20)) return false;
  const int64_t nnz = (int64_t)ip[n];
  if (nnz == 0) return false;
  const int64_t cols = std::max<int64_t>(int64_t(1) << 18, (n + 15) / 16);
  const unsigned nt = std::max(1u, std::min(16u, std::thread::hardware_concurrency()));
  std::vector<int64_t> far(nt, 0);
  std::vector<std::thread> th;
  for (unsigned t = 0; t < nt; ++t)
    th.emplace_back([&, t] {
      const int64_t r0 = n * t / nt, r1 = n * (t + 1) / nt;
      int64_t f = 0;
      for (int64_t r = r0; r < r1; ++r)
        for (int64_t e = ip[r]; e < ip[r + 1]; ++e) {
          const int64_t d = (int64_t)ix[e] - r;
          f += (d > cols / 2 || d < -cols / 2);
        }
      far[t] = f;
// ... 163 lines not shown
bool rs_build(int64_t n, const I *ip, const I *ix, const MV *dv, int64_t sell_slots, RsHost<MV> &p) {
  constexpr int H = kPairSlice;
  if (n == 0 || n >= (int64_t(1) << 28) - 1) return false;
  const int64_t ns = (n + H - 1) / H;
  p.width.assign(ns, 0);
  p.sptr.assign(ns + 1, 0);
  for (int64_t s = 0; s < ns; ++s) {
    int64_t w = 0;
    for (int64_t r = s * H; r < std::min<int64_t>(n, (s + 1) * H); ++r) w = std::max<int64_t>(w, ip[r + 1] - ip[r]);
    if (w > INT32_MAX / H) return false;
    p.width[s] = (int32_t)w;
    p.max_width = std::max(p.max_width, (int)w);
    p.sptr[s + 1] = p.sptr[s] + H * w;
  }
  const int64_t slots = p.sptr[ns];
  if (slots == 0 || slots * 4 > sell_slots * 5 + (int64_t)4 * H * p.max_width) return false;
  par_fill(p.colrank, slots + 2 * H, 0xFFFFFFFFu);
  par_fill(p.val, slots + 2 * H, MV(0));
  auto fill = [&](int64_t sa, int64_t sb) {
    std::vector<std::pair<int64_t, int>> run;
    for (int64_t s = sa; s < sb; ++s) {
      const int64_t r0 = s * H, r1 = std::min<int64_t>(n, r0 + H), base = p.sptr[s];
      for (int64_t r = r0; r < r1; ++r) {
        const int64_t e0 = (int64_t)ip[r], len = (int64_t)ip[r + 1] - e0;
        for (int64_t c0 = 0; c0 < len; c0 += kRsChunk) {
          const int m = (int)std::min<int64_t>(kRsChunk, len - c0);
          run.clear();
          for (int k = 0; k < m; ++k) run.emplace_back((int64_t)ix[e0 + c0 + k], k);
          std::stable_sort(run.begin(), run.end(),
                           [](const std::pair<int64_t, int> &x, const std::pair<int64_t, int> &y) { return x.first < y.first; });
          for (int j = 0; j < m; ++j) {
            const int64_t q = base + (c0 + j) * H + (r - r0);
            p.colrank[q] = (uint32_t)run[j].first | ((uint32_t)run[j].second << 28);
            p.val[q] = dv[e0 + c0 + run[j].second];
          }
        }
      }
    }
  };
  unsigned nt = std::max(1u, std::min(16u, std::thread::hardware_concurrency()));
  if (ns < 2048) nt = 1;
  std::vector<std::thread> th;
  for (unsigned t = 0; t < nt; ++t) th.emplace_back(fill, ns * t / nt, ns * (t + 1) / nt);
  for (auto &x : th) x.join();
  return true;
}

template <typename I>
static void dia_plan_host(int64_t n, int64_t nnz, const I *ip, const I *ix, int64_t *info, int32_t *widths,
                          int32_t *offsets, uint64_t *masks) {
  check_csr(n, nnz, ip, ix);
  int64_t ns = 0, sell_slots = 0, irr = 0;
  sell_plan(n, ip, nullptr, nullptr, &ns, &sell_slots, &irr);
  hvec<double> zeros;
  par_fill(zeros, (size_t)std::max<int64_t>(nnz, 1), 0.0);
  DiaHost<double> d;
  const bool built = dia_build(n, ip, ix, zeros.data(), sell_slots, d);
  info[0] = built ? 1 : 0;
  info[1] = built ? (int64_t)d.width.size() : 0;
  info[2] = built ? d.sptr.back() : 0;
  info[3] = built ? d.max_width : 0;
  if (!built) return;
  if (widths) std::copy(d.width.begin(), d.width.end(), widths);
  const int64_t cols = d.sptr.back() / kDiaSlice;
  if (offsets) std::copy(d.off.begin(), d.off.begin() + cols, offsets);
  if (masks) std::copy(d.mask.begin(), d.mask.begin() + 2 * cols, masks);
}

template <typename I, typename MV>
static void dia_uniform_plan_host(int64_t n, int64_t nnz, const I *ip, const I *ix, const MV *dv, int64_t *info,
                                  int32_t *flags, MV *values) {
  check_csr(n, nnz, ip, ix);
  int64_t ns = 0, sell_slots = 0, irr = 0;
  sell_plan(n, ip, nullptr, nullptr, &ns, &sell_slots, &irr);
  DiaHost<MV> d;
  const bool built = dia_build(n, ip, ix, dv, sell_slots, d);
  const int64_t cols = built ? d.sptr.back() / kDiaSlice : 0;
  info[0] = built ? 1 : 0;
  info[1] = cols;
  info[2] = built ? d.nuniform : 0;
  if (!built) return;
  if (flags) std::copy(d.uflag.begin(), d.uflag.begin() + cols, flags);
  if (values) std::memcpy(values, d.uval.data(), (size_t)cols * sizeof(MV));
}


template <typename I, typename MV>
bool cb_build(int64_t n, const I *ip, const I *ix, const MV *dv, CbHost<MV> &cb) {
  if (sizeof(I) != 4 || n * 8 < (int64_t(8) << 20)) return false;
  const int64_t nnz = (int64_t)ip[n];
  const char *cenv = getenv("KRY_CB_COLS");
  int64_t cols = cenv ? std::max<int64_t>(1024, atoll(cenv)) : std::max<int64_t>(int64_t(1) << 18, (n + 15) / 16);
  const int64_t nb = (n + cols - 1) / cols;
  if (nb < 2) return false;
  unsigned nt = std::max(1u, std::min(16u, std::thread::hardware_concurrency()));
  std::vector<int64_t> far(nt, 0);
  std::atomic<bool> sorted{true};
  {
    std::vector<std::thread> th;
    for (unsigned t = 0; t < nt; ++t)
      th.emplace_back([&, t] {
        const int64_t r0 = n * t / nt, r1 = n * (t + 1) / nt;
        int64_t f = 0;
        for (int64_t r = r0; r < r1; ++r)
          for (int64_t e = ip[r]; e < ip[r + 1]; ++e) {
            if (e > ip[r] && ix[e] < ix[e - 1]) sorted = false;
            const int64_t d = (int64_t)ix[e] - r;
            f += (d > cols / 2 || d < -cols / 2);
          }
        far[t] = f;
      });
    for (auto &x : th) x.join();
  }
  int64_t nfar = 0;
  for (int64_t f : far) nfar += f;
  if (!sorted || nnz == 0 || nfar * 4 < nnz) return false;
  const int64_t ng = (n + kCbRows - 1) / kCbRows;
  if (ng > 32 * 16384) return false;
  hvec<uint16_t> roff;
  par_fill(roff, nb * n + 256, (uint16_t)0);
  std::vector<int64_t> seg(nb * ng, 0);
  std::atomic<bool> fits{true};
  auto pass1 = [&](int64_t g0, int64_t g1) {
    std::vector<int64_t> cnt(nb);
    for (int64_t g = g0; g < g1; ++g) {
      std::fill(cnt.begin(), cnt.end(), 0);
      const int64_t r0 = g * kCbRows, r1 = std::min<int64_t>(n, r0 + kCbRows);
      for (int64_t r = r0; r < r1; ++r) {
        for (int64_t b = 0; b < nb; ++b) {
          if (cnt[b] > 65535) fits = false;
          roff[b * n + r] = (uint16_t)cnt[b];
        }
        for (int64_t e = ip[r]; e < ip[r + 1]; ++e) cnt[ix[e] / cols]++;
      }
      for (int64_t b = 0; b < nb; ++b) {
        if (cnt[b] > 65535) fits = false;
        seg[b * ng + g] = cnt[b];
      }
    }
  };
  std::vector<std::thread> th;
  for (unsigned t = 0; t < nt; ++t) th.emplace_back(pass1, ng * t / nt, ng * (t + 1) / nt);
  for (auto &x : th) x.join();
  th.clear();
  if (!fits) return false;
  cb.gptr.assign(nb * ng + 1, 0);
  for (int64_t i = 0; i < nb * ng; ++i) cb.gptr[i + 1] = cb.gptr[i] + seg[i];
  par_fill(cb.col, nnz + 256, (int32_t)0);
  par_fill(cb.val, nnz + 256, MV(0));
  auto pass2 = [&](int64_t g0, int64_t g1) {
    std::vector<int64_t> pos(nb);
    for (int64_t g = g0; g < g1; ++g) {
      for (int64_t b = 0; b < nb; ++b) pos[b] = cb.gptr[b * ng + g];
      const int64_t r0 = g * kCbRows, r1 = std::min<int64_t>(n, r0 + kCbRows);
      for (int64_t r = r0; r < r1; ++r)
        for (int64_t e = ip[r]; e < ip[r + 1]; ++e) {
          const int64_t p = pos[ix[e] / cols]++;
          cb.col[p] = (int32_t)ix[e];
          cb.val[p] = dv[e];
        }
    }
  };
  for (unsigned t = 0; t < nt; ++t) th.emplace_back(pass2, ng * t / nt, ng * (t + 1) / nt);
  for (auto &x : th) x.join();
  cb.nb = nb;
  cb.cols = cols;
// ... 245 lines not shown
                  "ILU(0) needs sorted rows without duplicates (row " + std::to_string(i) + ")");
      if (j <= i) lx.push_back(ix[e]);
      if (j == i) p.diag[(size_t)i] = e;
    }
    KRY_REQUIRE(p.diag[(size_t)i] >= 0, KRY_ESINGULAR, "singular matrix: no diagonal entry in row " + std::to_string(i));
    lp[(size_t)i + 1] = (I)lx.size();
  }
  tri_plan(n, (int64_t)lx.size(), lp.data(), lx.data(), true, p.tri);
}

template <typename I>
void color_plan(int64_t n, int64_t nnz, const I *ip, const I *ix, std::vector<int32_t> &color,
                std::vector<int32_t> &perm, int64_t *ncolors, int64_t *max_rows) {
  check_csr(n, nnz, ip, ix);
  KRY_REQUIRE(n < INT32_MAX, KRY_EUNSUPPORTED, "the colouring numbers rows in int32");
  std::vector<int64_t> tp((size_t)n + 1, 0);
  for (int64_t j = 0; j < n; ++j)
    for (int64_t e = (int64_t)ip[j]; e < (int64_t)ip[j + 1]; ++e)
      if ((int64_t)ix[e] > j) ++tp[(size_t)ix[e] + 1];
  for (int64_t c = 0; c < n; ++c) tp[(size_t)c + 1] += tp[(size_t)c];
  std::vector<int32_t> tx((size_t)tp[(size_t)n]);
  {
    std::vector<int64_t> next(tp.begin(), tp.end() - 1);
    for (int64_t j = 0; j < n; ++j)
      for (int64_t e = (int64_t)ip[j]; e < (int64_t)ip[j + 1]; ++e)
        if ((int64_t)ix[e] > j) tx[(size_t)next[(size_t)ix[e]]++] = (int32_t)j;
  }
  color.assign((size_t)n, 0);
  std::vector<int64_t> seen;
  std::vector<int32_t> count;
  for (int64_t i = 0; i < n; ++i) {
    for (int64_t e = (int64_t)ip[i]; e < (int64_t)ip[i + 1]; ++e)
      if ((int64_t)ix[e] < i) seen[(size_t)color[(size_t)ix[e]]] = i + 1;
    for (int64_t e = tp[(size_t)i]; e < tp[(size_t)i + 1]; ++e) seen[(size_t)color[(size_t)tx[(size_t)e]]] = i + 1;
    size_t c = 0;
    while (c < seen.size() && seen[c] == i + 1) ++c;
    if (c == seen.size()) {
      seen.push_back(0);
      count.push_back(0);
    }
    color[(size_t)i] = (int32_t)c;
    ++count[c];
  }
  *ncolors = (int64_t)count.size();
  *max_rows = 0;
  std::vector<int64_t> next(count.size() + 1, 0);
  for (size_t c = 0; c < count.size(); ++c) {
    *max_rows = std::max<int64_t>(*max_rows, count[c]);
    next[c + 1] = next[c] + count[c];
  }
  perm.assign((size_t)n, 0);
  for (int64_t i = 0; i < n; ++i) perm[(size_t)next[(size_t)color[(size_t)i]]++] = (int32_t)i;
}

#define KRY_HOST_I(I)                                                                                             \
  template void check_csr<I>(int64_t, int64_t, const I *, const I *);                                            \
  template bool scattered<I>(int64_t, const I *, const I *);                                                     \
  template bool rcm_order<I>(int64_t, const I *, const I *, int64_t, std::vector<int32_t> &, int64_t *);          \
  template void tri_plan<I>(int64_t, int64_t, const I *, const I *, bool, TriPlan &, const int32_t *);           \
  template void color_plan<I>(int64_t, int64_t, const I *, const I *, std::vector<int32_t> &,                   \
                              std::vector<int32_t> &, int64_t *, int64_t *);                                     \
  template void ilu0_plan<I>(int64_t, int64_t, const I *, const I *, Ilu0Plan &);                               \
  template void sell_plan<I>(int64_t, const I *, std::vector<int64_t> *, std::vector<int32_t> *, int64_t *,     \
                             int64_t *, int64_t *);                                                              \
  template bool compact_fill<I>(const std::vector<int64_t> &, const std::vector<int32_t> &, const hvec<I> &,     \
                                hvec<uint16_t> &, std::vector<int32_t> &);
#define KRY_HOST_IM(I, MV)                                                                                         \
  template void sell_fill<I, MV>(int64_t, const I *, const I *, const MV *, const std::vector<int64_t> &,       \
                                 const std::vector<int32_t> &, hvec<I> &, hvec<MV> &);                          \
  template bool dia_build<I, MV>(int64_t, const I *, const I *, const MV *, int64_t, DiaHost<MV> &, bool);      \
  template bool cb_build<I, MV>(int64_t, const I *, const I *, const MV *, CbHost<MV> &);                       \
  template bool pair_build<I, MV>(int64_t, const I *, const I *, const MV *, int64_t, PairHost<MV> &);          \
  template void renumber_csr<I, MV>(int64_t, const I *, const I *, const MV *, const std::vector<int32_t> &,    \
                                    hvec<I> &, hvec<I> &, hvec<MV> &);                                          \
  template bool rs_build<I, MV>(int64_t, const I *, const I *, const MV *, int64_t, RsHost<MV> &);              \
  template void tri_fill<I, MV>(const TriPlan &, const I *, const I *, const MV *, hvec<int32_t> &, hvec<MV> &,  \
                                hvec<int32_t> &, hvec<MV> &);
KRY_HOST_I(int32_t)
KRY_HOST_I(int64_t)
KRY_HOST_IM(int32_t, float)
KRY_HOST_IM(int32_t, double)
KRY_HOST_IM(int64_t, float)
KRY_HOST_IM(int64_t, double)
template void release_later<int32_t>(hvec<int32_t> &);
template void release_later<int64_t>(hvec<int64_t> &);
template void release_later<float>(hvec<float> &);
template void release_later<double>(hvec<double> &);
template void release_later<uint16_t>(hvec<uint16_t> &);
template void release_later<uint64_t>(hvec<uint64_t> &);
template void release_later<uint32_t>(hvec<uint32_t> &);

}

using namespace kry;

template <typename I>
static void rs_plan_host(int64_t n, int64_t nnz, const I *ip, const I *ix, int64_t *info, int32_t *widths,
                         uint32_t *colrank) {
  check_csr(n, nnz, ip, ix);
  int64_t ns = 0, sell_slots = 0, irr = 0;
  sell_plan(n, ip, nullptr, nullptr, &ns, &sell_slots, &irr);
  hvec<double> zeros;
  par_fill(zeros, (size_t)std::max<int64_t>(nnz, 1), 0.0);
  RsHost<double> r;
  const bool built = rs_build(n, ip, ix, zeros.data(), sell_slots, r);
  info[0] = built ? 1 : 0;
  info[1] = built ? (int64_t)r.width.size() : 0;
  info[2] = built ? r.sptr.back() : 0;
  info[3] = built ? r.max_width : 0;
  if (!built) return;
  if (widths) std::copy(r.width.begin(), r.width.end(), widths);
  if (colrank) std::copy(r.colrank.begin(), r.colrank.begin() + r.sptr.back(), colrank);
}

extern "C" {

const char *kry_last_error(void) { return kry::g_last_error.c_str(); }

int kry_csr_layout(int64_t n, const void *indptr, int itype, int64_t *nslices, int64_t *nslots,
                   int64_t *nirregular) {
  KRY_API_BEGIN
  KRY_REQUIRE(indptr && nslices && nslots && nirregular && n >= 0, KRY_EINVAL, "bad layout arguments");
  if (itype == KRY_I32)
    sell_plan(n, static_cast<const int32_t *>(indptr), nullptr, nullptr, nslices, nslots, nirregular);
  else if (itype == KRY_I64)
    sell_plan(n, static_cast<const int64_t *>(indptr), nullptr, nullptr, nslices, nslots, nirregular);
  else
    throw Error{KRY_EINVAL, "bad itype"};
  KRY_API_END
}

int kry_dia_plan(int64_t n, int64_t nnz, const void *indptr, const void *indices, int itype, int64_t *info,
                 int32_t *widths, int32_t *offsets, uint64_t *masks) {
  KRY_API_BEGIN
  KRY_REQUIRE(indptr && info && n >= 0 && nnz >= 0 && (nnz == 0 || indices), KRY_EINVAL, "bad plan arguments");
  if (itype == KRY_I32)
    dia_plan_host(n, nnz, static_cast<const int32_t *>(indptr), static_cast<const int32_t *>(indices), info, widths,
                  offsets, masks);
  else if (itype == KRY_I64)
    dia_plan_host(n, nnz, static_cast<const int64_t *>(indptr), static_cast<const int64_t *>(indices), info, widths,
                  offsets, masks);
  else
    throw Error{KRY_EINVAL, "bad itype"};
  KRY_API_END
}

int kry_dia_uniform_plan(int64_t n, int64_t nnz, const void *indptr, const void *indices, const void *data, int dtype,
                         int itype, int64_t *info, int32_t *flags, void *values) {
  KRY_API_BEGIN
  KRY_REQUIRE(indptr && info && n >= 0 && nnz >= 0 && (nnz == 0 || (indices && data)), KRY_EINVAL,
              "bad plan arguments");
  KRY_REQUIRE(dtype == KRY_F32 || dtype == KRY_F64, KRY_EINVAL, "dtype must be f32 or f64");
  KRY_REQUIRE(itype == KRY_I32 || itype == KRY_I64, KRY_EINVAL, "bad itype");
  static const double zd = 0;
  const void *dv = nnz ? data : (const void *)&zd;
  auto go = [&](auto *ip, auto *ix) {
    if (dtype == KRY_F64)
      dia_uniform_plan_host(n, nnz, ip, ix, static_cast<const double *>(dv), info, flags, static_cast<double *>(values));
    else
      dia_uniform_plan_host(n, nnz, ip, ix, static_cast<const float *>(dv), info, flags, static_cast<float *>(values));
  };
  if (itype == KRY_I32)
    go(static_cast<const int32_t *>(indptr), static_cast<const int32_t *>(indices));
  else
    go(static_cast<const int64_t *>(indptr), static_cast<const int64_t *>(indices));
  KRY_API_END
}

int kry_pair_plan(int64_t n, int64_t nnz, const void *indptr, const void *indices, int itype, int64_t *info,
                  int32_t *widths, int32_t *cbase, uint16_t *deltas) {
  KRY_API_BEGIN
  KRY_REQUIRE(indptr && info && n >= 0 && nnz >= 0 && (nnz == 0 || indices), KRY_EINVAL, "bad plan arguments");
  if (itype == KRY_I32)
    pair_plan_host(n, nnz, static_cast<const int32_t *>(indptr), static_cast<const int32_t *>(indices), info, widths,
                   cbase, deltas);
  else if (itype == KRY_I64)
    pair_plan_host(n, nnz, static_cast<const int64_t *>(indptr), static_cast<const int64_t *>(indices), info, widths,
                   cbase, deltas);
  else
    throw Error{KRY_EINVAL, "bad itype"};
  KRY_API_END
}

int kry_cb_plan(int64_t n, int64_t nnz, const void *indptr, const void *indices, int itype, int64_t *info,
                int64_t *gptr) {
  KRY_API_BEGIN
  KRY_REQUIRE(indptr && info && n >= 0 && nnz >= 0 && (nnz == 0 || indices), KRY_EINVAL, "bad plan arguments");
  if (itype == KRY_I32)
    cb_plan_host(n, nnz, static_cast<const int32_t *>(indptr), static_cast<const int32_t *>(indices), info, gptr);
  else if (itype == KRY_I64)
    cb_plan_host(n, nnz, static_cast<const int64_t *>(indptr), static_cast<const int64_t *>(indices), info, gptr);
  else
    throw Error{KRY_EINVAL, "bad itype"};
  KRY_API_END
}

int kry_rcm_plan(int64_t n, int64_t nnz, const void *indptr, const void *indices, int itype, int64_t wlimit,
                 int64_t *info, int32_t *perm) {
  KRY_API_BEGIN
  KRY_REQUIRE(indptr && info && n >= 0 && nnz >= 0 && (nnz == 0 || indices), KRY_EINVAL, "bad plan arguments");
  const int64_t wl = wlimit > 0 ? wlimit : std::max<int64_t>(int64_t(1) << 16, n / 32);
  std::vector<int32_t> p;
  int64_t levels = 0;
  bool built = false;
  if (itype == KRY_I32) {
    check_csr(n, nnz, static_cast<const int32_t *>(indptr), static_cast<const int32_t *>(indices));
    built = rcm_order(n, static_cast<const int32_t *>(indptr), static_cast<const int32_t *>(indices), wl, p, &levels);
  } else if (itype == KRY_I64) {
    check_csr(n, nnz, static_cast<const int64_t *>(indptr), static_cast<const int64_t *>(indices));
    built = rcm_order(n, static_cast<const int64_t *>(indptr), static_cast<const int64_t *>(indices), wl, p, &levels);
  } else {
    throw Error{KRY_EINVAL, "bad itype"};
  }
  info[0] = built ? 1 : 0;
  info[1] = built ? levels : 0;
  if (built && perm) std::copy(p.begin(), p.end(), perm);
  KRY_API_END
}

int kry_rs_plan(int64_t n, int64_t nnz, const void *indptr, const void *indices, int itype, int64_t *info,
                int32_t *widths, uint32_t *colrank) {
  KRY_API_BEGIN
  KRY_REQUIRE(indptr && info && n >= 0 && nnz >= 0 && (nnz == 0 || indices), KRY_EINVAL, "bad plan arguments");
  if (itype == KRY_I32)
    rs_plan_host(n, nnz, static_cast<const int32_t *>(indptr), static_cast<const int32_t *>(indices), info, widths,
                 colrank);
  else if (itype == KRY_I64)
    rs_plan_host(n, nnz, static_cast<const int64_t *>(indptr), static_cast<const int64_t *>(indices), info, widths,
                 colrank);
  else
    throw Error{KRY_EINVAL, "bad itype"};
  KRY_API_END
}

int kry_tri_plan_ordered(int64_t n, int64_t nnz, const void *indptr, const void *indices, int itype, int lower,
                         const int32_t *rank, int64_t *info, int32_t *level, int32_t *order, int32_t *launch,
                         int32_t *widths) {
  KRY_API_BEGIN
  KRY_REQUIRE(indptr && info && n >= 0 && nnz >= 0 && (nnz == 0 || indices), KRY_EINVAL, "bad plan arguments");
  TriPlan p;
  if (itype == KRY_I32)
    tri_plan(n, nnz, static_cast<const int32_t *>(indptr), static_cast<const int32_t *>(indices), lower != 0, p, rank);
  else if (itype == KRY_I64)
// ... 61 lines not shown
```

krylov_amd/csrc/host_image.hpp:

```cpp
#pragma once

#include <stdint.h>

#include <memory>
#include <utility>
#include <vector>

#include "host_common.hpp"

namespace kry {

template <class T>
struct NoInit : std::allocator<T> {
  template <class U>
  struct rebind {
    using other = NoInit<U>;
  };
  NoInit() = default;
  template <class U>
  NoInit(const NoInit<U> &) {}
  template <class U, class... A>
  void construct(U *q, A &&...a) {
    if constexpr (sizeof...(A) == 0) ::new ((void *)q) U;
    else ::new ((void *)q) U(std::forward<A>(a)...);
  }
};
template <class T>
using hvec = std::vector<T, NoInit<T>>;


template <class T>
void release_later(hvec<T> &v);

template <typename I>
void check_csr(int64_t n, int64_t nnz, const I *ip, const I *ix);

template <typename I>
void sell_plan(int64_t n, const I *ip, std::vector<int64_t> *sptr, std::vector<int32_t> *width, int64_t *nslices,
               int64_t *nslots, int64_t *nirr);
template <typename I, typename MV>
void sell_fill(int64_t n, const I *ip, const I *ix, const MV *dv, const std::vector<int64_t> &sptr,
               const std::vector<int32_t> &width, hvec<I> &sidx, hvec<MV> &sval);
template <typename I>
bool compact_fill(const std::vector<int64_t> &sptr, const std::vector<int32_t> &width, const hvec<I> &sidx,
                  hvec<uint16_t> &sdelta, std::vector<int32_t> &scbase);

template <typename MV>
struct DiaHost {
  std::vector<int64_t> sptr;
  std::vector<int32_t> width;
  std::vector<int32_t> off;
  hvec<uint64_t> mask;
  hvec<MV> val;
  int max_width = 0;
  std::vector<int32_t> uflag;
  std::vector<MV> uval;
  int64_t nuniform = 0;
};

template <typename I, typename MV>
bool dia_build(int64_t n, const I *ip, const I *ix, const MV *dv, int64_t sell_slots, DiaHost<MV> &d,
               bool uniform = true);

template <typename MV>
struct CbHost {
  int64_t nb = 0, cols = 0, ng = 0;
  std::vector<int64_t> gptr;
  hvec<uint16_t> roff;
  hvec<int32_t> col;
  hvec<MV> val;
};

template <typename I, typename MV>
bool cb_build(int64_t n, const I *ip, const I *ix, const MV *dv, CbHost<MV> &cb);

template <typename MV>
struct PairHost {
  std::vector<int64_t> sptr;
  std::vector<int32_t> width;
  std::vector<int32_t> cbase;
  hvec<uint16_t> delta;
  hvec<MV> val;
  int max_width = 0;
};

template <typename I, typename MV>
bool pair_build(int64_t n, const I *ip, const I *ix, const MV *dv, int64_t sell_slots, PairHost<MV> &p);

template <typename I>
bool rcm_order(int64_t n, const I *ip, const I *ix, int64_t wlimit, std::vector<int32_t> &perm, int64_t *levels);

template <typename I>
bool scattered(int64_t n, const I *ip, const I *ix);

template <typename I, typename MV>
void renumber_csr(int64_t n, const I *ip, const I *ix, const MV *dv, const std::vector<int32_t> &perm,
                  hvec<I> &ip2, hvec<I> &ix2, hvec<MV> &dv2);

template <typename MV>
struct RsHost {
  std::vector<int64_t> sptr;
  std::vector<int32_t> width;
  hvec<uint32_t> colrank;
  hvec<MV> val;
  int max_width = 0;
};
template <typename I, typename MV>
bool rs_build(int64_t n, const I *ip, const I *ix, const MV *dv, int64_t sell_slots, RsHost<MV> &r);

struct TriPlan {
  int64_t n = 0, nlevels = 0, nslices = 0, nslots = 0, max_level_rows = 0;
  std::vector<int32_t> level;
  std::vector<int32_t> order;
  std::vector<int32_t> lrow;
  std::vector<int32_t> lslice;
  std::vector<int32_t> swidth;
  std::vector<int64_t> sptr;
  std::vector<int32_t> launch;
  std::vector<int32_t> rank;
};
template <typename I>
void tri_plan(int64_t n, int64_t nnz, const I *ip, const I *ix, bool lower, TriPlan &p,
              const int32_t *rank = nullptr);
template <typename I, typename V>
void tri_fill(const TriPlan &p, const I *ip, const I *ix, const V *dv, hvec<int32_t> &rows, hvec<V> &diag,
              hvec<int32_t> &col, hvec<V> &val);

struct Ilu0Plan {
  TriPlan tri;
  std::vector<int64_t> diag;
};
template <typename I>
void ilu0_plan(int64_t n, int64_t nnz, const I *ip, const I *ix, Ilu0Plan &p);

template <typename I>
void color_plan(int64_t n, int64_t nnz, const I *ip, const I *ix, std::vector<int32_t> &color,
                std::vector<int32_t> &perm, int64_t *ncolors, int64_t *max_rows);

}
```

krylov_amd/csrc/objects.hpp:

```cpp
#pragma once

#include <utility>
#include <vector>

#include "common.hpp"

struct kry_ctx {
  int device = 0;
  hipStream_t stream = nullptr;
  hipEvent_t t0 = nullptr, t1 = nullptr;
  unsigned profile = 0;
  int prof_every = 1;
  int64_t prof_calls[4] = {0, 0, 0, 0};
  std::vector<std::pair<hipEvent_t, hipEvent_t>> ev_pool;
  size_t ev_used = 0;
  int ev_kernel_id = 0;
  int64_t prof_count[4] = {0, 0, 0, 0};
  double prof_ms[4] = {0, 0, 0, 0};
  std::vector<int> ev_ids;
  double *scratch = nullptr;
  size_t scratch_bytes = 0;
  void *pinned = nullptr;
  size_t pinned_bytes = 0;
};

struct kry_csr {
  kry_ctx *ctx = nullptr;
  int64_t n = 0, nnz = 0;
  int dtype = 0, itype = 0;
  int64_t nslices = 0, nslots = 0, nirregular = 0;
  int max_width = 0;
  void *sptr = nullptr;
  void *swidth = nullptr;
  void *sidx = nullptr;
  void *sval = nullptr;
  bool compact = false;
  void *sdelta = nullptr;
  void *scbase = nullptr;
  int64_t cb_nb = 0, cb_cols = 0, cb_ng = 0;
  void *cb_gptr = nullptr;
  void *cb_roff = nullptr;
  void *cb_col = nullptr;
  void *cb_val = nullptr;
  bool dia = false;
  int64_t dia_nslices = 0;
  int64_t dia_nslots = 0;
  int dia_max_width = 0;
  int dia_span = -1;
  void *dia_sptr = nullptr;
  void *dia_width = nullptr;
  void *dia_off = nullptr;
  void *dia_mask = nullptr;
  void *dia_val = nullptr;
  int64_t dia_nuniform = 0;
  void *dia_uflag = nullptr;
  void *dia_uval = nullptr;
  mutable int dia_lean = -1;
  bool sp = false;
  int64_t sp_nslices = 0, sp_nslots = 0;
  int sp_max_width = 0;
  void *sp_sptr = nullptr;
  void *sp_width = nullptr;
  void *sp_cbase = nullptr;
  void *sp_delta = nullptr;
  void *sp_val = nullptr;
  bool rs = false;
  int64_t rs_nslices = 0, rs_nslots = 0;
  int rs_max_width = 0;
  void *rs_sptr = nullptr;
  void *rs_width = nullptr;
  void *rs_colrank = nullptr;
  void *rs_val = nullptr;
  bool renumbered = false;
  std::vector<int32_t> perm_host;
  uint64_t perm_hash = 0;
  int64_t rcm_levels = 0;
  void *perm = nullptr;
  void *iperm = nullptr;
  void *indptr = nullptr;
  void *indices = nullptr;
  void *data = nullptr;
};

struct kry_vec {
  kry_ctx *ctx = nullptr;
  int64_t n = 0;
  int32_t k = 1;
  int dtype = 0;
  void *d = nullptr;
  size_t bytes() const { return (size_t)n * k * (dtype == KRY_F64 ? 8 : 4); }
};

namespace kry {

inline size_t dsize(int dtype) { return dtype == KRY_F64 ? 8 : 4; }
inline size_t isize(int itype) { return itype == KRY_I64 ? 8 : 4; }
inline size_t padded_elems(int64_t n, int k) { return ((size_t)n * k + 15) / 16 * 16; }

void *dev_alloc(size_t bytes);
void dev_free(void *p);
void mem_stats(int64_t *out);
void mem_release();
double *ctx_scratch(kry_ctx *ctx, size_t bytes);
void permute_rows(const kry_csr *A, const void *src, void *dst, int k, size_t esize, bool to_op, hipStream_t st);
void load_in(const kry_csr *A, const void *src, void *dst, int k, size_t esize, hipStream_t st);
void store_out(const kry_csr *A, const void *src, void *host, int k, size_t esize, hipStream_t st);
void host_xfer(void *dst, const void *src, size_t bytes, hipMemcpyKind kind, hipStream_t st);
bool env_off(const char *name);
struct DeviceCsrFlags {
  bool strictly_sorted = false, sorted = false, scattered = false;
};
template <typename MV>
int device_image_build(kry_csr *A, const int32_t *ip, const int32_t *ix, const MV *dv, bool renumber_candidates,
                       DeviceCsrFlags *out);
int rcm_order_device(kry_ctx *ctx, int64_t n, const int32_t *d_ip, const int32_t *d_ix, int64_t wlimit,
                     std::vector<int32_t> &perm, int64_t *levels);

struct ProfScope {
  kry_ctx *ctx;
  int id;
  hipEvent_t e1 = nullptr;
  ProfScope(kry_ctx *c, int kernel_id);
  ~ProfScope();
};

enum { PROF_SPMV = 0, PROF_UPDATE = 1, PROF_MGS = 2, PROF_OTHER = 3 };

}
```

krylov_amd/sparse.py:

```python
import ctypes
import weakref

import numpy as np
import scipy.sparse

from . import _lib
from ._lib import check, lib
from .device import DeviceVector, get_context


def _next_pow2(k):
    p = 1
    while p < k:
        p *= 2
    return p


class CsrOperator:

    def __init__(self, A, device=None, like=None, ctx=None, renumber=True):
        if isinstance(A, CsrOperator):
            raise TypeError("already a CsrOperator")
        if scipy.sparse.issparse(A):
            csr = A.tocsr() if A.format != "csr" else A
        elif isinstance(A, np.ndarray):
            if A.ndim != 2:
                raise ValueError("A must be 2-D")
            csr = scipy.sparse.csr_matrix(A)
        else:
            raise TypeError(
                f"cannot place {type(A).__name__} on the device: pass a scipy.sparse matrix, a dense "
                "ndarray, or a krylov_amd.CsrOperator (host-callback operators are not supported)"
            )
        if csr.shape[0] != csr.shape[1]:
            raise ValueError("A must be square")
        if np.iscomplexobj(csr.data):
            raise TypeError("complex matrices are outside the MI355X path (float32/float64 only)")
        dt = np.dtype(csr.dtype)
        if dt not in (np.float32, np.float64):
            dt = np.dtype(np.float64)
        self.ctx = get_context(device) if ctx is None else ctx
        self.shape = csr.shape
        self.dtype = dt
        self.n = csr.shape[0]
        self.nnz = int(csr.nnz)
        itype = np.int32 if (self.nnz < 2**31 and self.n < 2**31) else np.int64
        indptr = np.ascontiguousarray(csr.indptr, dtype=itype)
        indices = np.ascontiguousarray(csr.indices, dtype=itype)
        data = np.ascontiguousarray(csr.data, dtype=dt)
        self.index_dtype = np.dtype(itype)
        h = ctypes.c_void_p()
        if like is not None and like.renumbered and not renumber:
            raise ValueError("renumber=False and a renumbered `like` contradict each other")
        if like is not None and like.renumbered:
            if like.ctx is not self.ctx or like.n != self.n:
                raise ValueError("like: an operator of the same size on the same device")
            check(
                lib.kry_csr_create_like(
                    self.ctx.handle, like.handle, self.n, self.nnz, _lib.ptr(indptr), _lib.ptr(indices),
                    _lib.ptr(data), _lib.dtype_code(dt), _lib.itype_code(itype), ctypes.byref(h),
                )
            )
        elif not renumber:
            check(
                lib.kry_csr_create_ex(
                    self.ctx.handle, self.n, self.nnz, _lib.ptr(indptr), _lib.ptr(indices),
                    _lib.ptr(data), _lib.dtype_code(dt), _lib.itype_code(itype), 0, ctypes.byref(h),
                )
            )
        else:
            check(
                lib.kry_csr_create(
                    self.ctx.handle, self.n, self.nnz, _lib.ptr(indptr), _lib.ptr(indices),
                    _lib.ptr(data), _lib.dtype_code(dt), _lib.itype_code(itype), ctypes.byref(h),
                )
            )
        self.handle = h
        self._fin = _lib.own(self, lib.kry_csr_destroy, h)
        self.renumbered = self.layout()["renumbered"]

    @property
    def device(self):
        return self.ctx.device

    def layout(self):
        info = np.zeros(16, dtype=np.int64)
        check(lib.kry_csr_info_n(self.handle, info.ctypes.data_as(ctypes.POINTER(ctypes.c_int64)), 16))
        return {"slices": int(info[0]), "slots": int(info[1]), "irregular": int(info[2]), "compact": bool(info[3]),
                "col_blocks": int(info[4]), "dia": bool(info[5]), "dia_slots": int(info[6]), "pair": bool(info[7]),
                "pair_slots": int(info[8]), "rs": bool(info[9]), "rs_slots": int(info[10]),
                "renumbered": bool(info[11]), "rcm_levels": int(info[12]), "dia_uniform_cols": int(info[13]),
                "dia_value_bytes": int(info[14]), "dia_lean": bool(info[15])}

    def matvec_device(self, x, y):
        check(lib.kry_spmv(self.ctx.handle, self.handle, x.handle, y.handle))

    def matvec_op(self, x, y):
        check(lib.kry_spmv_op(self.ctx.handle, self.handle, x.handle, y.handle))

    def permute(self, src, dst, to_operator):
        check(lib.kry_csr_permute(self.ctx.handle, self.handle, src.handle, dst.handle, 1 if to_operator else 0))

    def __matmul__(self, x):
        x = np.asarray(x)
        if x.shape[0] != self.n:
            raise ValueError("dimension mismatch")
        dt = np.result_type(self.dtype, x.dtype)
        if dt not in (np.float32, np.float64):
            raise TypeError(f"unsupported vector dtype {x.dtype}")
        x2 = np.ascontiguousarray(x.reshape(self.n, -1), dtype=dt)
        k = x2.shape[1]
        kp = _next_pow2(k)
        if kp != k:
            x2 = np.concatenate([x2, np.zeros((self.n, kp - k), dtype=dt)], axis=1)
        xv = DeviceVector(self.ctx, self.n, kp, dt)
        xv.upload(x2)
        yv = DeviceVector(self.ctx, self.n, kp, dt)
        self.matvec_device(xv, yv)
        y = yv.to_host()[:, :k]
        return np.ascontiguousarray(y).reshape(x.shape)

    matvec = __matmul__

    def close(self):
        self._fin()

    def __repr__(self):
        return f"CsrOperator(n={self.n}, nnz={self.nnz}, dtype={self.dtype}, device={self.device})"


_CACHE_MAX = 4
_cache = {}


def _fingerprint(A):
    import xxhash

    h = xxhash.xxh3_64()
    if scipy.sparse.issparse(A):
        csr = A if A.format == "csr" else None
        if csr is None:
            return None
        for arr in (csr.indptr, csr.indices, csr.data):
            h.update(np.ascontiguousarray(arr).view(np.uint8).data)
        return (csr.shape, str(csr.dtype), str(csr.indices.dtype), csr.nnz, h.intdigest())
    if isinstance(A, np.ndarray):
        h.update(np.ascontiguousarray(A).view(np.uint8).data)
        return (A.shape, str(A.dtype), h.intdigest())
    return None


def clear_operator_cache():
    _cache.clear()
    _lib.empty_cache()


def as_device_operator(A, device=None, like=None, ctx=None):
    import os

    lk = like if (like is not None and like.renumbered) else None
    if isinstance(A, CsrOperator):
        if ctx is not None and A.ctx is not ctx:
            raise ValueError("the operator lives on another context than the solve")
        return A
    if ctx is not None and ctx is not get_context(ctx.device):
        return CsrOperator(A, like=lk, ctx=ctx)
    if os.environ.get("KRYLOV_CSR_CACHE", "1") == "0":
        return CsrOperator(A, device=device, like=lk)
    dev = get_context(device).device
    fp = _fingerprint(A)
    if fp is None:
        return CsrOperator(A, device=device, like=lk)
    key = (dev, id(A), None if lk is None else id(lk))
    hit = _cache.get(key)
    if (hit is not None and hit[0]() is A and hit[1] == fp
# ... 14 lines not shown
```

Measured before the change: 6564 CG iters/s (RHS-iterations/s over all GPUs).

## Deduplicate DIA slice descriptors into shared classes to shrink per-slice metadata

Hashes each DIA slice's column descriptor (offsets, masks, uniform flags and values), groups identical slices into classes, and stores one compact descriptor table per class plus a per-slice (first, width) word. The SpMV kernel reads the packed int2 word and indexes the class tables instead of per-slice sptr, width and full descriptor arrays, which should cut metadata traffic and make the descriptor tables small enough to stay cache-resident on a regular stencil. This adds host and device build passes with hashing and verification, plus env-var gating and a size cap.

Result: faster. 6965 CG iters/s (RHS-iterations/s over all GPUs) (median of 6 runs) (+6.1%).

```diff
diff --git a/include/krylov_hip.h b/include/krylov_hip.h
--- a/include/krylov_hip.h
+++ b/include/krylov_hip.h
@@ -67,11 +67,13 @@
                  int32_t *widths, int32_t *offsets, uint64_t *masks);
 int kry_dia_uniform_plan(int64_t n, int64_t nnz, const void *indptr, const void *indices, const void *data, int dtype,
                          int itype, int64_t *info, int32_t *flags, void *values);
+int kry_dia_class_plan(int64_t n, int64_t nnz, const void *indptr, const void *indices, const void *data, int dtype,
+                       int itype, int uniform, int64_t *info);
 int kry_pair_plan(int64_t n, int64_t nnz, const void *indptr, const void *indices, int itype, int64_t *info,
                   int32_t *widths, int32_t *cbase, uint16_t *deltas);
 int kry_cb_plan(int64_t n, int64_t nnz, const void *indptr, const void *indices, int itype, int64_t *info,
                 int64_t *gptr);
-#define KRY_CSR_INFO_LEN 16
+#define KRY_CSR_INFO_LEN 18
 int kry_csr_info_n(const kry_csr *A, int64_t *info, int32_t len);
 int kry_csr_info(const kry_csr *A, int64_t *info);
 
diff --git a/krylov_amd/_lib.py b/krylov_amd/_lib.py
--- a/krylov_amd/_lib.py
+++ b/krylov_amd/_lib.py
@@ -64,6 +64,7 @@
     "kry_csr_layout": [_i64, _vp, _int, _ip64, _ip64, _ip64],
     "kry_dia_plan": [ctypes.c_int64, ctypes.c_int64, _vp, _vp, _int, _ip64, _vp, _vp, _vp],
     "kry_dia_uniform_plan": [ctypes.c_int64, ctypes.c_int64, _vp, _vp, _vp, _int, _int, _ip64, _vp, _vp],
+    "kry_dia_class_plan": [ctypes.c_int64, ctypes.c_int64, _vp, _vp, _vp, _int, _int, _int, _ip64],
     "kry_pair_plan": [ctypes.c_int64, ctypes.c_int64, _vp, _vp, _int, _ip64, _vp, _vp, _vp],
     "kry_cb_plan": [ctypes.c_int64, ctypes.c_int64, _vp, _vp, _int, _ip64, _vp],
     "kry_csr_info": [_vp, _ip64],
@@ -282,6 +283,21 @@
     return {"cols": int(info[1]), "uniform": int(info[2]), "flags": flags, "values": values}
 
 
+def dia_class_plan(indptr, indices, data, uniform=True):
+    indptr = np.ascontiguousarray(indptr)
+    indices = np.ascontiguousarray(indices, dtype=indptr.dtype)
+    data = np.ascontiguousarray(data)
+    n, nnz = indptr.shape[0] - 1, indices.shape[0]
+    assert data.shape[0] == nnz
+    info = np.zeros(4, dtype=np.int64)
+    check(lib.kry_dia_class_plan(n, nnz, ptr(indptr), ptr(indices), ptr(data), dtype_code(data.dtype),
+                                 itype_code(indptr.dtype), 1 if uniform else 0,
+                                 info.ctypes.data_as(ctypes.POINTER(ctypes.c_int64))))
+    if not info[0]:
+        return None
+    return {"cols": int(info[1]), "classes": int(info[2]), "class_cols": int(info[3])}
+
+
 def pair_plan(indptr, indices):
     indptr = np.ascontiguousarray(indptr)
     indices = np.ascontiguousarray(indices, dtype=indptr.dtype)
diff --git a/krylov_amd/csrc/abi_core.hip b/krylov_amd/csrc/abi_core.hip
--- a/krylov_amd/csrc/abi_core.hip
+++ b/krylov_amd/csrc/abi_core.hip
@@ -386,7 +386,7 @@
 
 extern "C" {
 
-int kry_version(void) { return 111; }
+int kry_version(void) { return 112; }
 
 #ifndef KRY_BUILD_ID
 #define KRY_BUILD_ID "unknown"
@@ -471,7 +471,9 @@
                                          A->dia ? (A->dia_nslots / kDiaSlice - A->dia_nuniform) * kDiaSlice *
                                                       (int64_t)dsize(A->dtype)
                                                 : 0,
-                                         A->dia && dia_lean_on(A) ? 1 : 0};
+                                         A->dia && dia_lean_on(A) ? 1 : 0,
+                                         dia_classes_on(A) ? A->dia_ncls : 0,
+                                         dia_classes_on(A) ? A->dia_cls_cols : 0};
   for (int i = 0; i < len && i < KRY_CSR_INFO_LEN; ++i) info[i] = all[i];
   KRY_API_END
 }
@@ -632,6 +634,22 @@
       KRY_HIP(hipMemcpyAsync(A->dia_val, dh.val.data(), dh.val.size() * sizeof(MV), hipMemcpyHostToDevice, st));
       KRY_HIP(hipMemcpyAsync(A->dia_uflag, dh.uflag.data(), dh.uflag.size() * 4, hipMemcpyHostToDevice, st));
       KRY_HIP(hipMemcpyAsync(A->dia_uval, dh.uval.data(), dh.uval.size() * sizeof(MV), hipMemcpyHostToDevice, st));
+      DiaClassHost<MV> ch;
+      if (dia_classes(dh, ch)) {
+        A->dia_ncls = ch.nclasses;
+        A->dia_cls_cols = ch.ncols;
+        A->dia_cls_word = dev_alloc(ch.word.size() * 4 + 16);
+        A->dia_cls_off = dev_alloc(ch.off.size() * 4);
+        A->dia_cls_mask = dev_alloc(ch.mask.size() * 8);
+        A->dia_cls_uflag = dev_alloc(ch.uflag.size() * 4);
+        A->dia_cls_uval = dev_alloc(ch.uval.size() * sizeof(MV));
+        KRY_HIP(hipMemsetAsync(static_cast<char *>(A->dia_cls_word) + ch.word.size() * 4, 0, 16, st));
+        KRY_HIP(hipMemcpyAsync(A->dia_cls_word, ch.word.data(), ch.word.size() * 4, hipMemcpyHostToDevice, st));
+        KRY_HIP(hipMemcpyAsync(A->dia_cls_off, ch.off.data(), ch.off.size() * 4, hipMemcpyHostToDevice, st));
+        KRY_HIP(hipMemcpyAsync(A->dia_cls_mask, ch.mask.data(), ch.mask.size() * 8, hipMemcpyHostToDevice, st));
+        KRY_HIP(hipMemcpyAsync(A->dia_cls_uflag, ch.uflag.data(), ch.uflag.size() * 4, hipMemcpyHostToDevice, st));
+        KRY_HIP(hipMemcpyAsync(A->dia_cls_uval, ch.uval.data(), ch.uval.size() * sizeof(MV), hipMemcpyHostToDevice, st));
+      }
       KRY_HIP(hipStreamSynchronize(st));
       release_later(dh.val);
     }
@@ -727,7 +745,8 @@
                   A->cb_val, A->dia_sptr, A->dia_width, A->dia_off, A->dia_mask, A->dia_val,
                   A->sp_sptr, A->sp_width, A->sp_cbase, A->sp_delta, A->sp_val,
                   A->rs_sptr, A->rs_width, A->rs_colrank, A->rs_val, A->perm, A->iperm,
-                  A->dia_uflag, A->dia_uval};
+                  A->dia_uflag, A->dia_uval, A->dia_cls_word, A->dia_cls_off, A->dia_cls_mask,
+                  A->dia_cls_uflag, A->dia_cls_uval};
   for (void *b : bufs) dev_free(b);
 }
 
@@ -847,6 +866,20 @@
     note(A->dia_nuniform != B->dia_nuniform);
     buf(A->dia_uflag, B->dia_uflag, A->dia ? dc * 4 : 0);
     buf(A->dia_uval, B->dia_uval, A->dia ? dc * ds : 0);
+    const bool same_desc = nd == 0;
+    if (same_desc) {
+      note(A->dia_ncls != B->dia_ncls);
+      note(A->dia_cls_cols != B->dia_cls_cols);
+    }
+    if (same_desc && A->dia_ncls == B->dia_ncls && A->dia_cls_cols == B->dia_cls_cols) {
+      const int64_t cc = A->dia_cls_cols + kDiaPad;
+      const bool on = A->dia && A->dia_ncls > 0;
+      buf(A->dia_cls_word, B->dia_cls_word, on ? A->dia_nslices * 8 : 0);
+      buf(A->dia_cls_off, B->dia_cls_off, on ? cc * 4 : 0);
+      buf(A->dia_cls_mask, B->dia_cls_mask, on ? cc * 16 : 0);
+      buf(A->dia_cls_uflag, B->dia_cls_uflag, on ? cc * 4 : 0);
+      buf(A->dia_cls_uval, B->dia_cls_uval, on ? cc * ds : 0);
+    }
   }
   out[0] = nd;
   out[1] = mask;
diff --git a/krylov_amd/csrc/device.hpp b/krylov_amd/csrc/device.hpp
--- a/krylov_amd/csrc/device.hpp
+++ b/krylov_amd/csrc/device.hpp
@@ -521,6 +521,7 @@
 template <typename V, typename MV, int UNR, class Src, class Epi, int UNI = 1, bool LEAN = false>
 __global__ __launch_bounds__(kBlock) void spmv_dia_kernel(const int64_t *__restrict__ sptr,
                                                           const int *__restrict__ swidth,
+                                                          const int2 *__restrict__ cword,
                                                           const int *__restrict__ doff,
                                                           const uint64_t *__restrict__ dmask,
                                                           const int *__restrict__ duflag,
@@ -553,11 +554,22 @@
       dacc += epi(prow, 0, pend[0], bs(prow, 0));
     }
   };
+  int2 cnext = cword ? cword[s_begin] : int2{0, 0};
   for (int64_t s = s_begin; s < s_end; ++s) {
-    const int w = swidth[s];
-    const int64_t base = sptr[s];
+    int w;
+    int64_t c0;
+    [[maybe_unused]] int64_t base = 0;
+    if (cword) {
+      c0 = cnext.x;
+      w = cnext.y;
+      cnext = cword[s + 1];
+      if constexpr (UNI != 2) base = sptr[s];
+    } else {
+      w = swidth[s];
+      base = sptr[s];
+      c0 = base / kDiaSlice;
+    }
     const int64_t row = s * kDiaSlice + 2 * lane;
-    const int64_t c0 = base / kDiaSlice;
     const int *mo = doff + c0;
     const uint64_t *mk = dmask + 2 * c0;
     const int *mu = duflag + c0;
@@ -1444,6 +1456,18 @@
   return A->dia_lean == 1;
 }
 
+inline bool dia_classes_on(const kry_csr *A) {
+  if (A->dia_cls < 0) {
+    const char *e = getenv("KRY_DIA_CLASSES"), *m = getenv("KRY_DIA_CLASS_MAX_BYTES");
+    const int64_t cap = m ? std::min<int64_t>(kDiaClassMaxBytes, atoll(m)) : kDiaClassMaxBytes;
+    A->dia_cls = A->dia && A->dia_ncls > 0 && !(e && atoi(e) == 0) &&
+                         A->dia_cls_cols * dia_class_col_bytes(dsize(A->dtype)) <= cap
+                     ? 1
+                     : 0;
+  }
+  return A->dia_cls == 1;
+}
+
 template <typename I>
 inline bool spmv_column_blocked(const kry_csr *A, int k) {
   return sizeof(I) == 4 && k == 1 && !A->dia && A->cb_nb > 0;
@@ -1502,12 +1526,16 @@
                           : allu                             ? kDiaGridUniform
                                                              : kMaxGridBlk;
       grid = (int)std::max<int64_t>(1, std::min<int64_t>(dia_cap, (A->dia_nslices + 3) / 4));
+      const bool cls = dia_classes_on(A);
       auto go = [&](auto kern) {
         hipLaunchKernelGGL(kern, dim3(grid), dim3(kBlock), 0, st, static_cast<const int64_t *>(A->dia_sptr),
-                           static_cast<const int *>(A->dia_width), static_cast<const int *>(A->dia_off),
-                           static_cast<const uint64_t *>(A->dia_mask), static_cast<const int *>(A->dia_uflag),
-                           static_cast<const MV *>(A->dia_uval), static_cast<const MV *>(A->dia_val),
-                           A->dia_nslices, A->n, src, epi, part, ctrl, step);
+                           static_cast<const int *>(A->dia_width),
+                           static_cast<const int2 *>(cls ? A->dia_cls_word : nullptr),
+                           static_cast<const int *>(cls ? A->dia_cls_off : A->dia_off),
+                           static_cast<const uint64_t *>(cls ? A->dia_cls_mask : A->dia_mask),
+                           static_cast<const int *>(cls ? A->dia_cls_uflag : A->dia_uflag),
+                           static_cast<const MV *>(cls ? A->dia_cls_uval : A->dia_uval),
+                           static_cast<const MV *>(A->dia_val), A->dia_nslices, A->n, src, epi, part, ctrl, step);
       };
       if (dia_lean_on(A)) {
         if (allu) go(spmv_dia_kernel<V, MV, 8, Src, Epi, 2, true>);
diff --git a/krylov_amd/csrc/device_build.hip b/krylov_amd/csrc/device_build.hip
--- a/krylov_amd/csrc/device_build.hip
+++ b/krylov_amd/csrc/device_build.hip
@@ -1,4 +1,7 @@
 #include <hipcub/hipcub.hpp>
+
+#include <unordered_map>
+#include <vector>
 
 #include "common.hpp"
 #include "host_image.hpp"
@@ -238,6 +241,72 @@
   if (lane == 0 && nu) atomicAdd(nuniform, (unsigned long long)nu);
 }
 
+template <typename MV>
+__device__ inline uint64_t uval_bits(MV v) {
+  if constexpr (sizeof(MV) == 8) return (uint64_t)__double_as_longlong(v);
+  else return (uint64_t)__float_as_uint(v);
+}
+__device__ inline uint64_t hash_mix(uint64_t h, uint64_t v) {
+  h = (h ^ v) * 0x9E3779B97F4A7C15ull;
+  return h ^ (h >> 29);
+}
+template <typename MV>
+__global__ __launch_bounds__(kDb) void dia_class_hash_kernel(int64_t ns, const long long *__restrict__ sptr,
+                                                             const int *__restrict__ width,
+                                                             const int32_t *__restrict__ off,
+                                                             const uint64_t *__restrict__ mask,
+                                                             const int32_t *__restrict__ uflag,
+                                                             const MV *__restrict__ uval, uint64_t *__restrict__ hash) {
+  const int64_t s = (int64_t)blockIdx.x * kDb + threadIdx.x;
+  if (s >= ns) return;
+  const int64_t c0 = sptr[s] / kDiaSlice;
+  const int w = width[s];
+  uint64_t h = hash_mix(0x2545F4914F6CDD1Dull, (uint64_t)w);
+  for (int64_t j = c0; j < c0 + w; ++j) {
+    h = hash_mix(h, (uint32_t)off[j] | (uint64_t)(uint32_t)uflag[j] << 32);
+    h = hash_mix(h, mask[2 * j]);
+    h = hash_mix(h, mask[2 * j + 1]);
+    h = hash_mix(h, uval_bits(uval[j]));
+  }
+  hash[s] = h;
+}
+
+template <typename MV>
+__global__ __launch_bounds__(kDb) void dia_class_gather_kernel(
+    int64_t ncls, const long long *__restrict__ rep_c0, const int32_t *__restrict__ first,
+    const int32_t *__restrict__ cwidth, const int32_t *__restrict__ off, const uint64_t *__restrict__ mask,
+    const int32_t *__restrict__ uflag, const MV *__restrict__ uval, int32_t *__restrict__ toff,
+    uint64_t *__restrict__ tmask, int32_t *__restrict__ tuflag, MV *__restrict__ tuval) {
+  const int64_t k = (int64_t)blockIdx.x * kDb + threadIdx.x;
+  if (k >= ncls) return;
+  const int64_t c0 = rep_c0[k], t0 = first[k];
+  for (int j = 0; j < cwidth[k]; ++j) {
+    toff[t0 + j] = off[c0 + j];
+    tmask[2 * (t0 + j)] = mask[2 * (c0 + j)];
+    tmask[2 * (t0 + j) + 1] = mask[2 * (c0 + j) + 1];
+    tuflag[t0 + j] = uflag[c0 + j];
+    tuval[t0 + j] = uval[c0 + j];
+  }
+}
+
+template <typename MV>
+__global__ __launch_bounds__(kDb) void dia_class_verify_kernel(
+    int64_t ns, const long long *__restrict__ sptr, const int *__restrict__ width, const int32_t *__restrict__ word,
+    const int32_t *__restrict__ off, const uint64_t *__restrict__ mask, const int32_t *__restrict__ uflag,
+    const MV *__restrict__ uval, const int32_t *__restrict__ toff, const uint64_t *__restrict__ tmask,
+    const int32_t *__restrict__ tuflag, const MV *__restrict__ tuval, unsigned *bad) {
+  const int64_t s = (int64_t)blockIdx.x * kDb + threadIdx.x;
+  if (s >= ns) return;
+  const int64_t c0 = sptr[s] / kDiaSlice, t0 = word[2 * s];
+  const int w = width[s];
+  bool ok = word[2 * s + 1] == w;
+  for (int j = 0; j < w && ok; ++j)
+    ok = off[c0 + j] == toff[t0 + j] && mask[2 * (c0 + j)] == tmask[2 * (t0 + j)] &&
+         mask[2 * (c0 + j) + 1] == tmask[2 * (t0 + j) + 1] && uflag[c0 + j] == tuflag[t0 + j] &&
+         uval_bits(uval[c0 + j]) == uval_bits(tuval[t0 + j]);
+  if (!ok) atomicOr(bad, 1u);
+}
+
 int grid_for_n(int64_t items, int per_block) {
   return (int)std::max<int64_t>(1, std::min<int64_t>(1 << 20, (items + per_block - 1) / per_block));
 }
@@ -278,6 +347,75 @@
   KRY_HIP(hipMemcpyAsync(&v, d, sizeof(T), hipMemcpyDeviceToHost, st));
   KRY_HIP(hipStreamSynchronize(st));
   return v;
+}
+
+template <typename MV>
+void device_dia_classes(kry_csr *A, hipStream_t st) {
+  const int64_t ns = A->dia_nslices, cols = A->dia_nslots / kDiaSlice;
+  if (ns == 0) return;
+  const auto *sptr = static_cast<const long long *>(A->dia_sptr);
+  const auto *width = static_cast<const int *>(A->dia_width);
+  const auto *off = static_cast<const int32_t *>(A->dia_off);
+  const auto *mask = static_cast<const uint64_t *>(A->dia_mask);
+  const auto *uflag = static_cast<const int32_t *>(A->dia_uflag);
+  const auto *uval = static_cast<const MV *>(A->dia_uval);
+  Tmp dhash((size_t)ns * 8);
+  hipLaunchKernelGGL(dia_class_hash_kernel<MV>, dim3(grid_for_n(ns, kDb)), dim3(kDb), 0, st, ns, sptr, width, off, mask,
+                     uflag, uval, dhash.as<uint64_t>());
+  KRY_HIP(hipGetLastError());
+  std::vector<uint64_t> hash(ns);
+  std::vector<long long> hsptr(ns + 1);
+  std::vector<int32_t> hwidth(ns);
+  KRY_HIP(hipMemcpyAsync(hash.data(), dhash.p, (size_t)ns * 8, hipMemcpyDeviceToHost, st));
+  KRY_HIP(hipMemcpyAsync(hsptr.data(), sptr, (size_t)(ns + 1) * 8, hipMemcpyDeviceToHost, st));
+  KRY_HIP(hipMemcpyAsync(hwidth.data(), width, (size_t)ns * 4, hipMemcpyDeviceToHost, st));
+  KRY_HIP(hipStreamSynchronize(st));
+  const int64_t col_bytes = dia_class_col_bytes(sizeof(MV));
+  std::unordered_map<uint64_t, int32_t> cls_of;
+  std::vector<long long> rep_c0;
+  std::vector<int32_t> first, cwidth, word(2 * ns);
+  int64_t ccols = 0;
+  for (int64_t s = 0; s < ns; ++s) {
+    auto it = cls_of.find(hash[s]);
+    if (it == cls_of.end()) {
+      it = cls_of.emplace(hash[s], (int32_t)rep_c0.size()).first;
+      rep_c0.push_back(hsptr[s] / kDiaSlice);
+      first.push_back((int32_t)ccols);
+      cwidth.push_back(hwidth[s]);
+      ccols += hwidth[s];
+      if (ccols >= cols || ccols * col_bytes > kDiaClassMaxBytes) return;
+    }
+    word[2 * s] = first[it->second];
+    word[2 * s + 1] = cwidth[it->second];
+  }
+  const int64_t ncls = (int64_t)rep_c0.size(), tc = ccols + kDiaPad;
+  Tmp dword((size_t)ns * 8 + 16), toff((size_t)tc * 4), tmask((size_t)tc * 16), tuflag((size_t)tc * 4),
+      tuval((size_t)tc * sizeof(MV)), drep((size_t)ncls * 8), dfirst((size_t)ncls * 4), dcw((size_t)ncls * 4), dbad(16);
+  KRY_HIP(hipMemsetAsync(static_cast<char *>(dword.p) + (size_t)ns * 8, 0, 16, st));
+  KRY_HIP(hipMemsetAsync(toff.p, 0, (size_t)tc * 4, st));
+  KRY_HIP(hipMemsetAsync(tmask.p, 0, (size_t)tc * 16, st));
+  KRY_HIP(hipMemsetAsync(tuflag.p, 0, (size_t)tc * 4, st));
+  KRY_HIP(hipMemsetAsync(tuval.p, 0, (size_t)tc * sizeof(MV), st));
+  KRY_HIP(hipMemsetAsync(dbad.p, 0, 16, st));
+  KRY_HIP(hipMemcpyAsync(dword.p, word.data(), (size_t)ns * 8, hipMemcpyHostToDevice, st));
+  KRY_HIP(hipMemcpyAsync(drep.p, rep_c0.data(), (size_t)ncls * 8, hipMemcpyHostToDevice, st));
+  KRY_HIP(hipMemcpyAsync(dfirst.p, first.data(), (size_t)ncls * 4, hipMemcpyHostToDevice, st));
+  KRY_HIP(hipMemcpyAsync(dcw.p, cwidth.data(), (size_t)ncls * 4, hipMemcpyHostToDevice, st));
+  hipLaunchKernelGGL(dia_class_gather_kernel<MV>, dim3(grid_for_n(ncls, kDb)), dim3(kDb), 0, st, ncls,
+                     drep.as<const long long>(), dfirst.as<const int32_t>(), dcw.as<const int32_t>(), off, mask, uflag,
+                     uval, toff.as<int32_t>(), tmask.as<uint64_t>(), tuflag.as<int32_t>(), tuval.as<MV>());
+  hipLaunchKernelGGL(dia_class_verify_kernel<MV>, dim3(grid_for_n(ns, kDb)), dim3(kDb), 0, st, ns, sptr, width,
+                     dword.as<const int32_t>(), off, mask, uflag, uval, toff.as<const int32_t>(),
+                     tmask.as<const uint64_t>(), tuflag.as<const int32_t>(), tuval.as<const MV>(), dbad.as<unsigned>());
+  KRY_HIP(hipGetLastError());
+  if (read1(dbad.as<const unsigned>(), st) != 0) return;
+  A->dia_ncls = ncls;
+  A->dia_cls_cols = ccols;
+  A->dia_cls_word = dword.release();
+  A->dia_cls_off = toff.release();
+  A->dia_cls_mask = tmask.release();
+  A->dia_cls_uflag = tuflag.release();
+  A->dia_cls_uval = tuval.release();
 }
 
 }
@@ -397,6 +535,7 @@
         A->dia_val = dval.release();
         A->dia_uflag = duflag.release();
         A->dia_uval = duval.release();
+        device_dia_classes<MV>(A, st);
       }
     }
   }
diff --git a/krylov_amd/csrc/host_common.hpp b/krylov_amd/csrc/host_common.hpp
--- a/krylov_amd/csrc/host_common.hpp
+++ b/krylov_amd/csrc/host_common.hpp
@@ -13,6 +13,8 @@
 constexpr int kSlice = 64;
 constexpr int kDiaSlice = 128;
 constexpr int kDiaPad = 32;
+constexpr int64_t kDiaClassMaxBytes = int64_t(1) << 20;
+constexpr int64_t dia_class_col_bytes(size_t value_size) { return 4 + 16 + 4 + (int64_t)value_size; }
 constexpr int kPairSlice = 128;
 constexpr int kCbRows = 256;
 constexpr int kRsChunk = 16;
diff --git a/krylov_amd/csrc/host_image.cpp b/krylov_amd/csrc/host_image.cpp
--- a/krylov_amd/csrc/host_image.cpp
+++ b/krylov_amd/csrc/host_image.cpp
@@ -8,6 +8,7 @@
 #include <functional>
 #include <thread>
 #include <type_traits>
+#include <unordered_map>
 
 namespace kry {
 
@@ -276,6 +277,90 @@
   return true;
 }
 
+template <typename MV>
+bool dia_classes(const DiaHost<MV> &d, DiaClassHost<MV> &c) {
+  c = DiaClassHost<MV>();
+  const int64_t ns = (int64_t)d.width.size();
+  if (ns == 0) return false;
+  const int64_t cols = d.sptr[ns] / kDiaSlice;
+  std::vector<uint64_t> hash(ns);
+  auto mix = [](uint64_t h, uint64_t v) {
+    h = (h ^ v) * 0x9E3779B97F4A7C15ull;
+    return h ^ (h >> 29);
+  };
+  auto hpass = [&](int64_t sa, int64_t sb) {
+    for (int64_t s = sa; s < sb; ++s) {
+      const int64_t c0 = d.sptr[s] / kDiaSlice;
+      uint64_t h = mix(0x2545F4914F6CDD1Dull, (uint64_t)d.width[s]);
+      for (int64_t j = c0; j < c0 + d.width[s]; ++j) {
+        h = mix(h, (uint32_t)d.off[j] | (uint64_t)(uint32_t)d.uflag[j] << 32);
+        h = mix(h, d.mask[2 * j]);
+        h = mix(h, d.mask[2 * j + 1]);
+        h = mix(h, value_bits(d.uval[j]));
+      }
+      hash[s] = h;
+    }
+  };
+  {
+    unsigned nt = std::max(1u, std::min(16u, std::thread::hardware_concurrency()));
+    if (ns < 2048) nt = 1;
+    std::vector<std::thread> th;
+    for (unsigned t = 0; t < nt; ++t) th.emplace_back(hpass, ns * t / nt, ns * (t + 1) / nt);
+    for (auto &x : th) x.join();
+  }
+  auto same = [&](int64_t a, int64_t b) {
+    const int w = d.width[a];
+    if (w != d.width[b]) return false;
+    const int64_t ca = d.sptr[a] / kDiaSlice, cb = d.sptr[b] / kDiaSlice;
+    return std::memcmp(&d.off[ca], &d.off[cb], (size_t)w * 4) == 0 &&
+           std::memcmp(&d.mask[2 * ca], &d.mask[2 * cb], (size_t)w * 16) == 0 &&
+           std::memcmp(&d.uflag[ca], &d.uflag[cb], (size_t)w * 4) == 0 &&
+           std::memcmp(&d.uval[ca], &d.uval[cb], (size_t)w * sizeof(MV)) == 0;
+  };
+  const int64_t col_bytes = dia_class_col_bytes(sizeof(MV));
+  std::unordered_multimap<uint64_t, int32_t> bucket;
+  std::vector<int64_t> rep;
+  std::vector<int32_t> first;
+  std::vector<int32_t> cls(ns);
+  int64_t ccols = 0;
+  for (int64_t s = 0; s < ns; ++s) {
+    int32_t k = -1;
+    auto range = bucket.equal_range(hash[s]);
+    for (auto it = range.first; it != range.second && k < 0; ++it)
+      if (same(rep[it->second], s)) k = it->second;
+    if (k < 0) {
+      k = (int32_t)rep.size();
+      rep.push_back(s);
+      first.push_back((int32_t)ccols);
+      bucket.emplace(hash[s], k);
+      ccols += d.width[s];
+      if (ccols >= cols || ccols * col_bytes > kDiaClassMaxBytes) return false;
+    }
+    cls[s] = k;
+  }
+  if (ccols >= cols) return false;
+  c.nclasses = (int64_t)rep.size();
+  c.ncols = ccols;
+  c.word.resize(2 * ns);
+  for (int64_t s = 0; s < ns; ++s) {
+    c.word[2 * s] = first[cls[s]];
+    c.word[2 * s + 1] = d.width[s];
+  }
+  c.off.assign(ccols + kDiaPad, 0);
+  c.mask.assign(2 * (ccols + kDiaPad), 0);
+  c.uflag.assign(ccols + kDiaPad, 0);
+  c.uval.assign(ccols + kDiaPad, MV(0));
+  for (size_t k = 0; k < rep.size(); ++k) {
+    const int64_t c0 = d.sptr[rep[k]] / kDiaSlice;
+    const int w = d.width[rep[k]];
+    std::copy_n(&d.off[c0], w, &c.off[first[k]]);
+    std::copy_n(&d.mask[2 * c0], 2 * w, &c.mask[2 * (int64_t)first[k]]);
+    std::copy_n(&d.uflag[c0], w, &c.uflag[first[k]]);
+    std::copy_n(&d.uval[c0], w, &c.uval[first[k]]);
+  }
+  return true;
+}
+
 
 namespace {
 struct Team {
@@ -605,6 +690,22 @@
   if (!built) return;
   if (flags) std::copy(d.uflag.begin(), d.uflag.begin() + cols, flags);
   if (values) std::memcpy(values, d.uval.data(), (size_t)cols * sizeof(MV));
+}
+
+template <typename I, typename MV>
+static void dia_class_plan_host(int64_t n, int64_t nnz, const I *ip, const I *ix, const MV *dv, int uniform,
+                                int64_t *info) {
+  check_csr(n, nnz, ip, ix);
+  int64_t ns = 0, sell_slots = 0, irr = 0;
+  sell_plan(n, ip, nullptr, nullptr, &ns, &sell_slots, &irr);
+  DiaHost<MV> d;
+  const bool built = dia_build(n, ip, ix, dv, sell_slots, d, uniform != 0);
+  DiaClassHost<MV> c;
+  const bool cls = built && dia_classes(d, c);
+  info[0] = built ? 1 : 0;
+  info[1] = built ? d.sptr.back() / kDiaSlice : 0;
+  info[2] = cls ? c.nclasses : 0;
+  info[3] = cls ? c.ncols : 0;
 }
 
 
@@ -1016,6 +1117,8 @@
 KRY_HOST_IM(int32_t, double)
 KRY_HOST_IM(int64_t, float)
 KRY_HOST_IM(int64_t, double)
+template bool dia_classes<float>(const DiaHost<float> &, DiaClassHost<float> &);
+template bool dia_classes<double>(const DiaHost<double> &, DiaClassHost<double> &);
 template void release_later<int32_t>(hvec<int32_t> &);
 template void release_later<int64_t>(hvec<int64_t> &);
 template void release_later<float>(hvec<float> &);
@@ -1093,6 +1196,26 @@
       dia_uniform_plan_host(n, nnz, ip, ix, static_cast<const double *>(dv), info, flags, static_cast<double *>(values));
     else
       dia_uniform_plan_host(n, nnz, ip, ix, static_cast<const float *>(dv), info, flags, static_cast<float *>(values));
+  };
+  if (itype == KRY_I32)
+    go(static_cast<const int32_t *>(indptr), static_cast<const int32_t *>(indices));
+  else
+    go(static_cast<const int64_t *>(indptr), static_cast<const int64_t *>(indices));
+  KRY_API_END
+}
+
+int kry_dia_class_plan(int64_t n, int64_t nnz, const void *indptr, const void *indices, const void *data, int dtype,
+                       int itype, int uniform, int64_t *info) {
+  KRY_API_BEGIN
+  KRY_REQUIRE(indptr && info && n >= 0 && nnz >= 0 && (nnz == 0 || (indices && data)), KRY_EINVAL,
+              "bad plan arguments");
+  KRY_REQUIRE(dtype == KRY_F32 || dtype == KRY_F64, KRY_EINVAL, "dtype must be f32 or f64");
+  KRY_REQUIRE(itype == KRY_I32 || itype == KRY_I64, KRY_EINVAL, "bad itype");
+  static const double zd = 0;
+  const void *dv = nnz ? data : (const void *)&zd;
+  auto go = [&](auto *ip, auto *ix) {
+    if (dtype == KRY_F64) dia_class_plan_host(n, nnz, ip, ix, static_cast<const double *>(dv), uniform, info);
+    else dia_class_plan_host(n, nnz, ip, ix, static_cast<const float *>(dv), uniform, info);
   };
   if (itype == KRY_I32)
     go(static_cast<const int32_t *>(indptr), static_cast<const int32_t *>(indices));
diff --git a/krylov_amd/csrc/host_image.hpp b/krylov_amd/csrc/host_image.hpp
--- a/krylov_amd/csrc/host_image.hpp
+++ b/krylov_amd/csrc/host_image.hpp
@@ -61,6 +61,18 @@
 template <typename I, typename MV>
 bool dia_build(int64_t n, const I *ip, const I *ix, const MV *dv, int64_t sell_slots, DiaHost<MV> &d,
                bool uniform = true);
+
+template <typename MV>
+struct DiaClassHost {
+  int64_t nclasses = 0, ncols = 0;
+  std::vector<int32_t> word;
+  std::vector<int32_t> off;
+  std::vector<uint64_t> mask;
+  std::vector<int32_t> uflag;
+  std::vector<MV> uval;
+};
+template <typename MV>
+bool dia_classes(const DiaHost<MV> &d, DiaClassHost<MV> &c);
 
 template <typename MV>
 struct CbHost {
diff --git a/krylov_amd/csrc/objects.hpp b/krylov_amd/csrc/objects.hpp
--- a/krylov_amd/csrc/objects.hpp
+++ b/krylov_amd/csrc/objects.hpp
@@ -56,6 +56,14 @@
   void *dia_uflag = nullptr;
   void *dia_uval = nullptr;
   mutable int dia_lean = -1;
+  int64_t dia_ncls = 0;
+  int64_t dia_cls_cols = 0;
+  void *dia_cls_word = nullptr;
+  void *dia_cls_off = nullptr;
+  void *dia_cls_mask = nullptr;
+  void *dia_cls_uflag = nullptr;
+  void *dia_cls_uval = nullptr;
+  mutable int dia_cls = -1;
   bool sp = false;
   int64_t sp_nslices = 0, sp_nslots = 0;
   int sp_max_width = 0;
diff --git a/krylov_amd/sparse.py b/krylov_amd/sparse.py
--- a/krylov_amd/sparse.py
+++ b/krylov_amd/sparse.py
@@ -84,13 +84,14 @@
         return self.ctx.device
 
     def layout(self):
-        info = np.zeros(16, dtype=np.int64)
-        check(lib.kry_csr_info_n(self.handle, info.ctypes.data_as(ctypes.POINTER(ctypes.c_int64)), 16))
+        info = np.zeros(18, dtype=np.int64)
+        check(lib.kry_csr_info_n(self.handle, info.ctypes.data_as(ctypes.POINTER(ctypes.c_int64)), 18))
         return {"slices": int(info[0]), "slots": int(info[1]), "irregular": int(info[2]), "compact": bool(info[3]),
                 "col_blocks": int(info[4]), "dia": bool(info[5]), "dia_slots": int(info[6]), "pair": bool(info[7]),
                 "pair_slots": int(info[8]), "rs": bool(info[9]), "rs_slots": int(info[10]),
                 "renumbered": bool(info[11]), "rcm_levels": int(info[12]), "dia_uniform_cols": int(info[13]),
-                "dia_value_bytes": int(info[14]), "dia_lean": bool(info[15])}
+                "dia_value_bytes": int(info[14]), "dia_lean": bool(info[15]),
+                "dia_classes": int(info[16]), "dia_class_cols": int(info[17])}
 
     def matvec_device(self, x, y):
         check(lib.kry_spmv(self.ctx.handle, self.handle, x.handle, y.handle))
```
